# redwarp/kmeans-gpu

Hardware: AMD Instinct MI355X
Metric: pixels/sec per Lloyd iteration (8192x8192, k=256) (higher is better)
Workload: dtype f32; 1 GPU; synthetic uniform RGBA 8192x8192 (seed 0x5EED0003), k=256, one Lloyd iteration = update + assign (labels written every iteration) + accumulate; width=8192, height=8192, k=256, collective_backend=none (one rank), collective_ranks=1, label_pass=before the next iteration, update=by the last launch of the assign pass (kmg_lloyd_assign_update)

## Files before the change

### kmeans-gpu_amd/csrc/kmg_cube.hip

```cpp

#include "kmg_internal.h"
#include "kmg_table_dev.h"

#include <hip/hip_fp16.h>
#include <stdlib.h>

namespace kmg {

typedef float f32x2 __attribute__((ext_vector_type(2)));


namespace {

constexpr uint32_t kMaxListed = 32;
constexpr uint32_t kMaxLong = 256;
constexpr uint32_t kLongFlag = 0x200u;

__device__ __forceinline__ uint32_t sel3(uint32_t i, uint32_t x0, uint32_t x1, uint32_t x2)
{
    return i == 0u ? x0 : (i == 1u ? x1 : x2);
}

__device__ __forceinline__ int round_dir(int g, int m)
{
    const int a = g < 0 ? -g : g;
    const int r = (4 * a >= 3 * m ? 1 : 0) + (4 * a >= m ? 1 : 0);
    return g < 0 ? -r : r;
}

typedef unsigned short u16x2 __attribute__((ext_vector_type(2)));

__device__ __forceinline__ uint32_t group8_or(uint32_t v)
{
    v |= dpp_u32<kDppXor1>(v);
    v |= dpp_u32<kDppXor2>(v);
    v |= dpp_u32<kDppHalfMirror>(v);
    return v;
}

__device__ __forceinline__ uint32_t group8_min_u32(uint32_t v)
{
    v = min(v, dpp_u32<kDppXor1>(v));
    v = min(v, dpp_u32<kDppXor2>(v));
    v = min(v, dpp_u32<kDppHalfMirror>(v));
    return v;
}

__device__ __forceinline__ uint32_t group8_max_u32(uint32_t v)
{
    v = max(v, dpp_u32<kDppXor1>(v));
    v = max(v, dpp_u32<kDppXor2>(v));
    v = max(v, dpp_u32<kDppHalfMirror>(v));
    return v;
}



__device__ __forceinline__ uint32_t cell_pair_entry(const uint32_t idx[8], uint32_t occ, uint32_t lane)
{
    uint32_t rem = occ;
    uint32_t lab0 = 0, lab1 = 0, lab2 = 0, cnt0 = 0, cnt1 = 0, cnt2 = 0, msk0 = 0, msk1 = 0, msk2 = 0, n_occ = 0;
#pragma unroll
    for (int t = 0; t < 3; ++t) {
        const unsigned long long any = __ballot(rem != 0u);
        if (any) {
            uint32_t mine = 0;
#pragma unroll
            for (int q = 7; q >= 0; --q) mine = ((rem >> q) & 1u) ? idx[q] : mine;
            const uint32_t v = lane_value(mine, (uint32_t)__builtin_ctzll(any));
            uint32_t mm = 0;
#pragma unroll
            for (int q = 0; q < 8; ++q) mm |= (idx[q] == v ? 1u : 0u) << q;
            mm &= rem;
            rem &= ~mm;
            const uint32_t packed = wave_add_u32((uint32_t)__builtin_popcount(mm) | (t == 0 ? (uint32_t)__builtin_popcount(occ) << 10 : 0u));
            const uint32_t c = packed & 1023u;
            if (t == 0) { lab0 = v; msk0 = mm; cnt0 = c; n_occ = packed >> 10; }
            if (t == 1) { lab1 = v; msk1 = mm; cnt1 = c; }
            if (t == 2) { lab2 = v; msk2 = mm; cnt2 = c; }
        }
    }
    uint32_t a = 0;
    if (cnt1 > cnt0) a = 1;
    if (cnt2 > sel3(a, cnt0, cnt1, cnt2)) a = 2;
    uint32_t b = a == 0u ? 1u : 0u;
    if (a != 1u && b != 1u && cnt1 > sel3(b, cnt0, cnt1, cnt2)) b = 1;
    if (a != 2u && cnt2 > sel3(b, cnt0, cnt1, cnt2)) b = 2;
    const uint32_t labA = sel3(a, lab0, lab1, lab2), labB = sel3(b, lab0, lab1, lab2);
    const uint32_t mA = sel3(a, msk0, msk1, msk2), mB = sel3(b, msk0, msk1, msk2);
    const uint32_t rest = occ & ~mA;
    const uint32_t nA = sel3(a, cnt0, cnt1, cnt2), nR = n_occ - nA;
    if (nR == 0u) return pair_entry(labA, labA, 0u, 0u, 0u);

    const uint32_t half = ((lane >> 5) & 1u) | (((lane >> 4) & 1u) << 10) | (((lane >> 3) & 1u) << 20);
    const uint32_t hR = wave_add_u32((uint32_t)__builtin_popcount(rest) * half);
    const uint32_t hA = wave_add_u32((uint32_t)__builtin_popcount(mA) * half);
    const int gx = (int)((hR & 1023u) * nA) - (int)((hA & 1023u) * nR);
    const int gy = (int)(((hR >> 10) & 1023u) * nA) - (int)(((hA >> 10) & 1023u) * nR);
    const int gz = (int)((hR >> 20) * nA) - (int)((hA >> 20) * nR);
    const int ax = gx < 0 ? -gx : gx, ay = gy < 0 ? -gy : gy, az = gz < 0 ? -gz : gz;
    const int m = ax > ay ? (ax > az ? ax : az) : (ay > az ? ay : az);
    int nx = 2, ny = 0, nz = 0;
    if (m > 0) { nx = round_dir(gx, m); ny = round_dir(gy, m); nz = round_dir(gz, m); }

    const int xl = (int)(((lane >> 5) & 1u) * 4u + ((lane >> 1) & 3u));
    const int yl = (int)(((lane >> 4) & 1u) * 4u + (lane & 1u) * 2u);
    const int zl = (int)(((lane >> 3) & 1u) * 4u);
    const int bias = 7 * ((nx < 0 ? -nx : 0) + (ny < 0 ? -ny : 0) + (nz < 0 ? -nz : 0));
    const int p0 = nx * xl + ny * yl + nz * zl + bias;
    int p[8];
#pragma unroll
    for (int q = 0; q < 8; ++q) p[q] = p0 + ny * (q >> 2) + nz * (q & 3);
    const uint32_t notB = occ & ~mB;
    uint32_t tl = 63u, hi = 64u;
#pragma unroll
    for (int q = 0; q < 8; ++q) {
        if ((rest >> q) & 1u) tl = min(tl, (uint32_t)p[q]);
        if ((notB >> q) & 1u) hi = min(hi, (uint32_t)(63 - p[q]));
    }
    u16x2 packed = __builtin_bit_cast(u16x2, tl | (hi << 16));
    packed = __builtin_elementwise_min(packed, __builtin_bit_cast(u16x2, dpp_u32<kDppXor1>(__builtin_bit_cast(uint32_t, packed))));
    packed = __builtin_elementwise_min(packed, __builtin_bit_cast(u16x2, dpp_u32<kDppXor2>(__builtin_bit_cast(uint32_t, packed))));
    packed = __builtin_elementwise_min(packed, __builtin_bit_cast(u16x2, dpp_u32<kDppHalfMirror>(__builtin_bit_cast(uint32_t, packed))));
    packed = __builtin_elementwise_min(packed, __builtin_bit_cast(u16x2, dpp_u32<kDppMirror>(__builtin_bit_cast(uint32_t, packed))));
    packed = __builtin_elementwise_min(packed, __builtin_bit_cast(u16x2, (uint32_t)__builtin_amdgcn_update_dpp(-1, (int)__builtin_bit_cast(uint32_t, packed), 0x142, 0xA, 0xF, false)));
    packed = __builtin_elementwise_min(packed, __builtin_bit_cast(u16x2, (uint32_t)__builtin_amdgcn_update_dpp(-1, (int)__builtin_bit_cast(uint32_t, packed), 0x143, 0xC, 0xF, false)));
    const uint32_t pk = lane_value(__builtin_bit_cast(uint32_t, packed), 63);
    const int tlo = (int)(pk & 0xFFFFu);
    const int thi = 63 - (int)(pk >> 16);
    const int w = thi + 1 > tlo ? thi + 1 - tlo : 0;
    const uint32_t code = pair_dir_code(nx, ny, nz);
    if (w <= 6) return pair_entry(labA, labB, code, (uint32_t)tlo, (uint32_t)w);
    uint32_t low = 0, high = 0;
#pragma unroll
    for (int q = 0; q < 8; ++q) {
        if ((occ >> q) & 1u) { low += p[q] < tlo ? 1u : 0u; high += p[q] > thi ? 1u : 0u; }
    }
    const uint32_t lh = wave_add_u32(low | (high << 10));
    if ((lh & 1023u) >= (lh >> 10)) return pair_entry(labA, labB, code, (uint32_t)tlo, 7u);
    const int range = 7 * ((nx < 0 ? -nx : nx) + (ny < 0 ? -ny : ny) + (nz < 0 ? -nz : nz));
    return pair_entry(labB, labA, pair_dir_code(-nx, -ny, -nz), (uint32_t)(range - thi), 7u);
}

__device__ __forceinline__ uint32_t merge_state(uint32_t a, uint32_t b)
{
    return (a == kSubEmpty) ? b : ((b == kSubEmpty || b == a) ? a : (uint32_t)kSubMixed);
}

template <typename LabelT>
__device__ __forceinline__ void store_labels64(LabelT *dst64, uint32_t label, uint32_t lane)
{
    if (sizeof(LabelT) == 1) {
        const uint32_t t = label | (dpp_u32<kDppXor1>(label) << 8);
        const uint32_t u = t | (dpp_u32<kDppXor2>(t) << 16);
        if ((lane & 3u) == 0u) reinterpret_cast<uint32_t *>(dst64)[lane >> 2] = u;
    } else {
        const uint32_t t = label | (dpp_u32<kDppXor1>(label) << 16);
        if ((lane & 1u) == 0u) reinterpret_cast<uint32_t *>(dst64)[lane >> 1] = t;
    }
}


struct alignas(16) CellWork {
    uint16_t list[kMaxListed];
    unsigned long long br[4];
    uint32_t npop;
    uint32_t scan_set;
    uint32_t pad[6];
};
static_assert(sizeof(CellWork) == 128, "CellWork layout");

constexpr uint32_t kPairPending = 0xFFFFFFFEu;

constexpr uint32_t kLongSegs = 16, kLongSegCap = kCells / kLongSegs, kLongCount = 0, kLongCells = 64;
constexpr size_t kListsWords = kLongCells + kCells;
constexpr uint32_t kItemCands = 12;

__device__ __forceinline__ void flush_bins(const unsigned long long *bins, uint32_t k, uint32_t repl, uint32_t bin_stride,
                                           int64_t *sums, uint32_t n_rows)
{
    __syncthreads();
    unsigned long long *row = reinterpret_cast<unsigned long long *>(sums) + (uint64_t)(blockIdx.x % n_rows) * 4ull * k;
    for (uint32_t i = threadIdx.x; i < 4u * k; i += blockDim.x) {
        unsigned long long v = 0ull;
        for (uint32_t r = 0; r < repl; ++r) v += bins[(uint64_t)r * bin_stride + i];
        if (v) atomicAdd(row + i, v);
    }
}

__device__ __forceinline__ uint2 long_list_stage(const float4 *s_cent, const unsigned long long *s_masks, uint16_t *s_long,
                                              unsigned long long *s_sub, float4 sb0, float4 sb1, float4 sb2, uint32_t npop,
                                              uint32_t words, uint64_t *sub_masks_cell)
{
    const uint32_t lane = threadIdx.x & 63u;
    const uint32_t sub_of_lane = lane >> 3, cand_of_lane = lane & 7u;
    uint32_t base = 0;
    for (uint32_t w = 0; w < words; ++w) {
        const unsigned long long m = uniform_u64(s_masks[w]);
        if ((m >> lane) & 1ull) s_long[base + bits_below_lane(m)] = (uint16_t)(w * 64u + lane);
        base += (uint32_t)__builtin_popcountll(m);
    }
    if (lane < 32u) s_sub[lane] = 0ull;
    __builtin_amdgcn_wave_barrier();
    CellBounds sb;
    sb.L0 = sb0.x; sb.L1 = sb0.y; sb.a0 = sb0.z; sb.a1 = sb0.w;
    sb.b0 = sb1.x; sb.b1 = sb1.y; sb.C0 = sb1.z; sb.C1 = sb1.w;
    sb.wC0 = sb2.x; sb.wC1 = sb2.y; sb.wH0 = sb2.z; sb.wH1 = sb2.w;
    const uint32_t rounds = (npop + 7u) >> 3;
    float Usub = 3.0e38f;
    for (uint32_t r = 0; r < rounds; ++r) {
        const uint32_t pos = r * 8u + cand_of_lane;
        if (pos < npop) {
            const float4 c = s_cent[s_long[pos]];
            Usub = fminf(Usub, key_range(sb, c.x, c.y, c.z, c.w).hi);
        }
    }
    const float Us = mask_threshold(group8_min(Usub));
    for (uint32_t r = 0; r < rounds; ++r) {
        const uint32_t pos = r * 8u + cand_of_lane;
        if (pos < npop) {
            const uint32_t j = s_long[pos];
            const float4 c = s_cent[j];
            if (key_range(sb, c.x, c.y, c.z, c.w).lo <= Us) atomicOr(&s_sub[sub_of_lane * 4u + (j >> 6)], 1ull << (j & 63u));
        }
    }
    __builtin_amdgcn_wave_barrier();
    const unsigned long long mine = lane < 32u ? s_sub[lane] : 0ull;
    if (lane < 32u) sub_masks_cell[lane] = mine;
    uint32_t cnt = (uint32_t)__builtin_popcountll(mine);
    uint32_t one = mine ? (lane & 3u) * 64u + (uint32_t)__builtin_ctzll(mine) : 0u;
    cnt += dpp_u32<kDppXor1>(cnt); one += dpp_u32<kDppXor1>(one);
    cnt += dpp_u32<kDppXor2>(cnt); one += dpp_u32<kDppXor2>(one);
    uint2 r;
    r.x = (uint32_t)__builtin_amdgcn_ds_bpermute((int)((lane * 4u) << 2), (int)cnt);
    r.y = (uint32_t)__builtin_amdgcn_ds_bpermute((int)((lane * 4u) << 2), (int)one);
    return r;
}


constexpr uint32_t kAffineFloats = 24;
struct HalfModel {
    uint32_t q[kAffineFloats];
    __device__ __forceinline__ float operator[](int i) const
    {
        if (i >= 42) return bits_to_float(q[21 + (i - 42)]);
        const uint32_t h = (i & 1) ? q[i >> 1] >> 16 : q[i >> 1] & 0xFFFFu;
        return __half2float(__ushort_as_half((unsigned short)h));
    }
    __device__ __forceinline__ void load(const float *table, uint64_t sub_cell)
    {
        const uint4 *mp = reinterpret_cast<const uint4 *>(table + sub_cell * kAffineFloats);
#pragma unroll
        for (int t = 0; t < 6; ++t) {
            const uint4 v = mp[t];
            q[4 * t] = v.x; q[4 * t + 1] = v.y; q[4 * t + 2] = v.z; q[4 * t + 3] = v.w;
// ... 484 lines not shown
                }
                const float thr0 = tie_threshold(best0), thr1 = tie_threshold(best1);
                const bool near0 = second0 <= thr0, near1 = second1 <= thr1;
                if (__ballot(near0 || near1)) {
                    float lb0 = 100000.0f, lb1 = 100000.0f;
                    uint32_t li0 = 0u, li1 = 0u;
                    for (uint32_t w = 0; w < (k + 63u) / 64u; ++w) {
                        for (unsigned long long m = cand_word(w); m; m &= m - 1ull) {
                            const uint32_t j = w * 64u + (uint32_t)__builtin_ctzll(m);
                            const float4 c = s_cent[j];
                            if (near0 && cie94_key(pt0, c.x, c.y, c.z, c.w) <= thr0) {
                                const float d = cie94_c(v0.x, v0.y, v0.z, v0.w, c.x, c.y, c.z, c.w);
                                if (d < lb0) { lb0 = d; li0 = j; }
                            }
                            if (near1 && cie94_key(pt1, c.x, c.y, c.z, c.w) <= thr1) {
                                const float d = cie94_c(v1.x, v1.y, v1.z, v1.w, c.x, c.y, c.z, c.w);
                                if (d < lb1) { lb1 = d; li1 = j; }
                            }
                        }
                    }
                    ix0 = near0 ? li0 : ix0;
                    ix1 = near1 ? li1 : ix1;
                }
            }
            auto finish = [&](uint32_t s, uint32_t ix, uint32_t cnt, float vL, float va, float vb) {
                s_lbl[s * 64u + lane] = (LabelT)ix;
                label_set |= 1u << s;
                const bool counts = cnt != 0u;
                const unsigned long long occm = __ballot(counts);
                uint32_t st = kSubEmpty;
                if (occm) {
                    const uint32_t X0 = lane_value(ix, (uint32_t)__builtin_ctzll(occm));
                    const unsigned long long other = __ballot(counts && ix != X0);
                    uint32_t R = X0;
                    if (other) {
                        const uint32_t X1 = lane_value(ix, (uint32_t)__builtin_ctzll(other));
                        if (__builtin_popcountll(__ballot(counts && ix == X1)) > __builtin_popcountll(occm & ~other)) R = X1;
                    }
                    st = other ? (uint32_t)kSubMixed : X0;
                    if (SUMS) {
                        if ((lane >> 2) == s) atomicAdd(bins + 4ull * R + (lane & 3u), (unsigned long long)sagg);
                        if (other && counts && ix != R) {
                            const long long m = (long long)cnt;
                            const long long c0 = m * (long long)lab_fix(vL), c1 = m * (long long)lab_fix(va), c2 = m * (long long)lab_fix(vb);
                            unsigned long long *to = my_bins + 4ull * ix, *from = my_bins + 4ull * R;
                            atomicAdd(to + 0, (unsigned long long)c0); atomicAdd(from + 0, (unsigned long long)(-c0));
                            atomicAdd(to + 1, (unsigned long long)c1); atomicAdd(from + 1, (unsigned long long)(-c1));
                            atomicAdd(to + 2, (unsigned long long)c2); atomicAdd(from + 2, (unsigned long long)(-c2));
                            atomicAdd(to + 3, (unsigned long long)m);  atomicAdd(from + 3, (unsigned long long)(-m));
                        }
                    }
                }
                if (sizeof(LabelT) != 1 && lane == 0u) sub[s] = (uint16_t)st;
            };
            finish(s0, ix0, cnt0, v0.x, v0.y, v0.z);
            if (s1 < 8u) finish(s1, ix1, cnt1, v1.x, v1.y, v1.z);
        };
        for (;;) {
            KMG_REQUEST_COLOURS(B);
            scan_pair(A_s0, A_s1, A_v0, A_v1, A_c0, A_c1);
            if (B_s0 >= 8u) break;
            KMG_REQUEST_COLOURS(A);
            scan_pair(B_s0, B_s1, B_v0, B_v1, B_c0, B_c1);
            if (A_s0 >= 8u) break;
        }
#undef KMG_REQUEST_COLOURS
        __builtin_amdgcn_wave_barrier();
        if ((label_set >> (lane >> 3)) & 1u) {
            if (sizeof(LabelT) == 1)
                *reinterpret_cast<uint2 *>(cell_labels + lane * 8u) = *reinterpret_cast<const uint2 *>(s_lbl + lane * 8u);
            else
                *reinterpret_cast<uint4 *>(cell_labels + lane * 8u) = *reinterpret_cast<const uint4 *>(s_lbl + lane * 8u);
        }
        __builtin_amdgcn_wave_barrier();
    }
    if (SUMS) flush_bins(bins, k, repl, bin_stride, sums, n_rows);
}

template <typename LabelT>
__global__ __launch_bounds__(kBlock) void k_cube_pairs(const uint32_t *__restrict__ work, int with_work,
                                                       const uint8_t *__restrict__ occ_bits,
                                                       const LabelT *__restrict__ colour_labels,
                                                       uint16_t *__restrict__ sub_table, uint32_t flags,
                                                       int64_t *__restrict__ sums, uint32_t k, CubeTail tail)
{
    if (tail.acc_out && blockIdx.x == gridDim.x - 1u) {
        __shared__ uint32_t s_count;
        for (uint32_t i = threadIdx.x; i < 4u * k; i += kBlock) tail.acc_out[i] = sums[i];
        if (tail.do_update) update_centroids(sums, k, tail.convergence, tail.cent, tail.n_converged, &s_count, kBlock);
        __syncthreads();
        for (uint32_t i = threadIdx.x; i < 4u * k; i += kBlock) sums[i] = 0;
    }
    if (flags & kCubeNoEntries) return;
    const uint32_t lane = threadIdx.x & 63;
    const uint32_t wave = __builtin_amdgcn_readfirstlane(blockIdx.x * (kBlock / 64) + (threadIdx.x >> 6));
    const uint32_t n_waves = gridDim.x * (kBlock / 64);
    const uint32_t n_work = with_work ? __builtin_amdgcn_readfirstlane(work[0]) : kCells;
    const uint32_t *cells = with_work ? work + 1 : nullptr;
    for (uint32_t wi = wave; wi < n_work; wi += n_waves) {
        const uint32_t cell = cells ? __builtin_amdgcn_readfirstlane(cells[wi]) : wi;
        if (sizeof(LabelT) == 1) {
            uint32_t *pair_entry_ptr = reinterpret_cast<uint32_t *>(sub_table + kSubCells + kCells) + cell;
            if (__builtin_amdgcn_readfirstlane(*pair_entry_ptr) != kPairPending) continue;
            const uint2 lv = *reinterpret_cast<const uint2 *>(colour_labels + (uint64_t)cell * kCellColours + lane * 8u);
            const uint32_t occ = occ_bits ? (uint32_t)occ_bits[(uint64_t)cell * 64u + lane] : 0xFFu;
            uint32_t idx[8];
#pragma unroll
            for (uint32_t q = 0; q < 4u; ++q) { idx[q] = (lv.x >> (8u * q)) & 0xFFu; idx[4u + q] = (lv.y >> (8u * q)) & 0xFFu; }
            const uint32_t e = cell_pair_entry(idx, occ, lane);
            if (lane == 0u) *pair_entry_ptr = e;
        } else {
            uint32_t st = lane < 8u ? (uint32_t)sub_table[cell * 8u + lane] : (uint32_t)kSubEmpty;
#pragma unroll
            for (int off = 1; off < 8; off <<= 1) st = merge_state(st, (uint32_t)__shfl_xor(st, off, 64));
            if (lane == 0u) sub_table[kSubCells + cell] = (uint16_t)st;
        }
    }
}

constexpr uint32_t kSmallMaxK = kCubeSmallMaxK;
constexpr uint32_t kSmallRepl = 16;
constexpr int kSmallBlock = 512;
constexpr uint32_t kSmallWaves = kSmallBlock / 64;
constexpr uint32_t kSmallCells = kSmallWaves * 8u;
constexpr uint32_t kSmallEmit = 0x100u;
constexpr uint32_t kSmallTests = 2048;

__device__ __forceinline__ void affine_features(const float4 v, double F[7])
{
    const PixelTerms p = pixel_terms_c(v.x, v.y, v.z, v.w);
    F[0] = (double)p.L; F[1] = (double)p.wC; F[2] = (double)p.wC * (double)p.C;
    F[3] = (double)p.wH * (double)p.a; F[4] = (double)p.wH * (double)p.b; F[5] = (double)p.wH * (double)p.C; F[6] = (double)p.wH;
}

__global__ __launch_bounds__(kBlock) void k_sub_affine(const float4 *__restrict__ lab_table,
                                                       const CellBounds *__restrict__ sub_bounds, float *__restrict__ affine)
{
    const uint32_t sc = blockIdx.x * kBlock + threadIdx.x;
    if (sc >= kSubCells) return;
    const float4 *col = lab_table + (uint64_t)sc * 64u;
    double S0[7], Sx[7], Sy[7], Sz[7];
#pragma unroll
    for (int m = 0; m < 7; ++m) S0[m] = Sx[m] = Sy[m] = Sz[m] = 0.0;
    for (uint32_t q = 0; q < 64u; ++q) {
        double F[7];
        affine_features(col[q], F);
        const double dx = (double)((q >> 4) & 3u) - 1.5, dy = (double)((q >> 2) & 3u) - 1.5, dz = (double)(q & 3u) - 1.5;
#pragma unroll
        for (int m = 0; m < 7; ++m) { S0[m] += F[m]; Sx[m] += F[m] * dx; Sy[m] += F[m] * dy; Sz[m] += F[m] * dz; }
    }
    float al[7], bx[7], by[7], bz[7];
    double rmin[7], rmax[7];
#pragma unroll
    for (int m = 0; m < 7; ++m) {
        al[m] = __half2float(__float2half_rn((float)(S0[m] / 64.0))); bx[m] = __half2float(__float2half_rn((float)(Sx[m] / 80.0)));
        by[m] = __half2float(__float2half_rn((float)(Sy[m] / 80.0))); bz[m] = __half2float(__float2half_rn((float)(Sz[m] / 80.0)));
        rmin[m] = 1.0e300; rmax[m] = -1.0e300;
    }
    for (uint32_t q = 0; q < 64u; ++q) {
        double F[7];
        affine_features(col[q], F);
        const double dx = (double)((q >> 4) & 3u) - 1.5, dy = (double)((q >> 2) & 3u) - 1.5, dz = (double)(q & 3u) - 1.5;
#pragma unroll
        for (int m = 0; m < 7; ++m) {
            const double r = F[m] - ((double)al[m] + ((double)bx[m] * dx + ((double)by[m] * dy + (double)bz[m] * dz)));
            rmin[m] = fmin(rmin[m], r); rmax[m] = fmax(rmax[m], r);
        }
    }
    uint32_t *out = reinterpret_cast<uint32_t *>(affine) + (uint64_t)sc * kAffineFloats;
    unsigned short h[42];
#pragma unroll
    for (int m = 0; m < 7; ++m) {
        const double pad = 1.0e-12 * (fabs((double)al[m]) + 1.5 * (fabs((double)bx[m]) + fabs((double)by[m]) + fabs((double)bz[m])) + 1.0);
        const double lo = rmin[m] - pad, hi = rmax[m] + pad;
        float flo = (float)lo, fhi = (float)hi;
        if ((double)flo > lo) flo = nextafterf(flo, -3.0e38f);
        if ((double)fhi < hi) fhi = nextafterf(fhi, 3.0e38f);
        h[6 * m + 0] = __half_as_ushort(__float2half_rn(al[m])); h[6 * m + 1] = __half_as_ushort(__float2half_rn(bx[m]));
        h[6 * m + 2] = __half_as_ushort(__float2half_rn(by[m])); h[6 * m + 3] = __half_as_ushort(__float2half_rn(bz[m]));
        h[6 * m + 4] = __half_as_ushort(__float2half_rd(flo)); h[6 * m + 5] = __half_as_ushort(__float2half_ru(fhi));
    }
#pragma unroll
    for (int w = 0; w < 21; ++w) out[w] = (uint32_t)h[2 * w] | ((uint32_t)h[2 * w + 1] << 16);
    out[21] = float_to_bits(sub_bounds[sc].C1);
    out[22] = float_to_bits(sub_bounds[sc].wH1);
    out[23] = 0u;
}

size_t sub_affine_bytes() { return sizeof(float) * (size_t)kAffineFloats * kSubCells; }

hipError_t launch_sub_affine(const float4 *lab_table, const CellBounds *sub_bounds, float *affine, hipStream_t st)
{
    hipLaunchKernelGGL(k_sub_affine, dim3(kSubCells / kBlock), dim3(kBlock), 0, st, lab_table, sub_bounds, affine);
    return hipGetLastError();
}

template <int KP, bool SUMS>
__global__ __launch_bounds__(kSmallBlock) __attribute__((amdgpu_waves_per_eu(4, 4))) void k_cube_small(const uint32_t *__restrict__ hist, const int64_t *__restrict__ agg,
                                                            const int64_t *__restrict__ sub_agg,
                                                            const uint8_t *__restrict__ occ_bits,
                                                            const uint32_t *__restrict__ work,
                                                            const CellBounds *__restrict__ bounds,
                                                            const CellBounds *__restrict__ sub_bounds,
                                                            const float *__restrict__ sub_affine,
                                                            const Centroid *__restrict__ cent, uint32_t k,
                                                            const float4 *__restrict__ lab_table,
                                                            uint64_t *__restrict__ masks_out,
                                                            CellWork *__restrict__ cell_work,
                                                            uint8_t *__restrict__ colour_labels,
                                                            uint16_t *__restrict__ sub_table,
                                                            int64_t *__restrict__ sums, uint32_t n_rows, uint32_t flags,
                                                            unsigned long long *__restrict__ stats)
{
    extern __shared__ float4 smem4[];
    float4 *s_cent = smem4;
    unsigned long long *bins = reinterpret_cast<unsigned long long *>(smem4 + KP);
    const uint32_t bin_stride = 4u * k + 4u;
    const uint32_t n_bins = SUMS ? kSmallRepl * bin_stride : 0u;
    uint8_t *s_lbl = reinterpret_cast<uint8_t *>(bins + n_bins);
    uint32_t *s_mask = reinterpret_cast<uint32_t *>(s_lbl + kSmallCells * kCellColours);
    float *s_U = reinterpret_cast<float *>(s_mask + kSmallBlock);
    uint32_t *s_cell = reinterpret_cast<uint32_t *>(s_U + kSmallBlock);
    uint32_t *s_count = s_cell + kSmallCells;
    uint16_t *s_ent = reinterpret_cast<uint16_t *>(s_count + 4);
    uint16_t *s_pend = s_ent + kSmallBlock;
    uint16_t *s_test = s_pend + kSmallCells;
    uint8_t *s_istar = reinterpret_cast<uint8_t *>(s_test + kSmallTests);
    const uint32_t n_work_v = SUMS ? work[opaque_vgpr_zero()] : kCells;
    for (uint32_t i = threadIdx.x; i < (uint32_t)KP; i += kSmallBlock) {
        float4 v = make_float4(1.0e18f, 0.0f, 0.0f, 0.0f);
        if (i < k) { const Centroid c = cent[i]; v = make_float4(c.L, c.a, c.b, c.C); }
        s_cent[i] = v;
    }
    for (uint32_t i = threadIdx.x; i < n_bins; i += kSmallBlock) bins[i] = 0ull;
    if (threadIdx.x < 4u) s_count[threadIdx.x] = 0u;
    __syncthreads();
    if (threadIdx.x < k) {
        const float4 c = s_cent[threadIdx.x];
        if (!(fabsf(c.x) <= 1024.0f && fabsf(c.y) <= 1024.0f && fabsf(c.z) <= 1024.0f)) s_count[2] = 1u;
    }
    __syncthreads();
    const bool dominance = sub_affine != nullptr && s_count[2] == 0u;

    const uint32_t lane = threadIdx.x & 63u, wv = threadIdx.x >> 6;
    unsigned long long *my_bins = bins + (uint64_t)(lane & (kSmallRepl - 1u)) * bin_stride;
    uint32_t *pair_entries = reinterpret_cast<uint32_t *>(sub_table + kSubCells + kCells);
    const uint32_t ci = lane >> 3, sub = lane & 7u, slot = wv * 8u + ci;
    unsigned long long st_single = 0, st_multi = 0, st_decided = 0, st_scanned = 0, st_cands = 0;

    const uint32_t n_work = __builtin_amdgcn_readfirstlane(n_work_v);
    const uint32_t tasks = (n_work + 7u) >> 3;
    for (uint32_t base = blockIdx.x * kSmallWaves; base < tasks; base += gridDim.x * kSmallWaves) {
        const uint32_t task = base + wv;
        const uint32_t pos = task + ci * tasks;
        const bool valid = task < tasks && pos < n_work;
        const uint32_t cell = valid ? ((SUMS && n_work != kCells) ? work[1u + pos] : pos) : 0u;
        const uint32_t sc = cell * 8u + sub;
        const float4 *cbp = reinterpret_cast<const float4 *>(bounds + cell);
        const float4 cb0 = cbp[0], cb1 = cbp[1], cb2 = cbp[2];
        const float4 *sbp = reinterpret_cast<const float4 *>(sub_bounds + sc);
        const float4 sb0 = sbp[0], sb1 = sbp[1], sb2 = sbp[2];
        longlong2 s01 = {0, 0}, s23 = {0, 1};
        long long cell_sum = 0;
        if (SUMS) {
            const longlong2 *sp = reinterpret_cast<const longlong2 *>(sub_agg + (uint64_t)sc * 4u);
            s01 = sp[0]; s23 = sp[1];
            cell_sum = agg[4ull * cell + (sub & 3u)];
        }
        const bool occupied = valid && s23.y != 0;
        uint32_t mask = 0u;
        {
            CellBounds cb;
            cb.L0 = cb0.x; cb.L1 = cb0.y; cb.a0 = cb0.z; cb.a1 = cb0.w;
            cb.b0 = cb1.x; cb.b1 = cb1.y; cb.C0 = cb1.z; cb.C1 = cb1.w;
            cb.wC0 = cb2.x; cb.wC1 = cb2.y; cb.wH0 = cb2.z; cb.wH1 = cb2.w;
            constexpr int PER = KP / 8;
            float lo[PER], Uc = 3.0e38f;
#pragma unroll
            for (int q = 0; q < PER; ++q) {
                const float4 c = s_cent[sub * PER + q];
                const KeyRange kr = key_range(cb, c.x, c.y, c.z, c.w);
                lo[q] = kr.lo;
                Uc = fminf(Uc, kr.hi);
            }
            const float Ucs = mask_threshold(group8_min(Uc));
            uint32_t bits = 0u;
#pragma unroll
            for (int q = 0; q < PER; ++q) bits |= (lo[q] <= Ucs ? 1u : 0u) << (sub * PER + q);
            const uint32_t cmask = group8_or(bits);
            CellBounds sb;
            sb.L0 = sb0.x; sb.L1 = sb0.y; sb.a0 = sb0.z; sb.a1 = sb0.w;
            sb.b0 = sb1.x; sb.b1 = sb1.y; sb.C0 = sb1.z; sb.C1 = sb1.w;
            sb.wC0 = sb2.x; sb.wC1 = sb2.y; sb.wH0 = sb2.z; sb.wH1 = sb2.w;
            float U = 3.0e38f;
            uint32_t istar = 0u;
            for (uint32_t m = cmask; m; m &= m - 1u) {
                const uint32_t j = (uint32_t)__builtin_ctz(m);
                const float4 c = s_cent[j];
                const float hi = key_range(sb, c.x, c.y, c.z, c.w).hi;
                istar = hi < U ? j : istar;
                U = fminf(U, hi);
            }
            const float Us = mask_threshold(U);
            for (uint32_t m = cmask; m; m &= m - 1u) {
                const uint32_t j = (uint32_t)__builtin_ctz(m);
                const float4 c = s_cent[j];
                mask |= (key_range(sb, c.x, c.y, c.z, c.w).lo <= Us ? 1u : 0u) << j;
            }
            s_mask[threadIdx.x] = mask;
            const uint32_t others = mask & ~(1u << istar);
            if (dominance && occupied && others) {
                s_U[threadIdx.x] = U;
                s_istar[threadIdx.x] = (uint8_t)istar;
                const uint32_t nt = (uint32_t)__builtin_popcount(others);
                uint32_t at = atomicAdd(&s_count[3], nt);
                for (uint32_t m = others; m && at < kSmallTests; m &= m - 1u, ++at)
                    s_test[at] = (uint16_t)((threadIdx.x << 5) | (uint32_t)__builtin_ctz(m));
            }
        }
        if (sub == 0u) s_cell[slot] = cell;
        __syncthreads();
        if (dominance) {
            const uint32_t n_tests = min(s_count[3], kSmallTests);
            for (uint32_t t = threadIdx.x; t < n_tests; t += kSmallBlock) {
                const uint32_t e = (uint32_t)s_test[t] >> 5, j = (uint32_t)s_test[t] & 31u;
                const uint32_t tsc = s_cell[e >> 3] * 8u + (e & 7u);
                HalfModel mdl;
                mdl.load(sub_affine, tsc);
                if (dominated(mdl, s_cent[j], s_cent[s_istar[e]], s_U[e])) atomicAnd(&s_mask[e], ~(1u << j));
            }
            __syncthreads();
            mask = s_mask[threadIdx.x];
        }

        const uint32_t np = (uint32_t)__builtin_popcount(mask);
        const bool decided = occupied && np == 1u, scan = occupied && np > 1u;
        const uint32_t X = (uint32_t)__builtin_ctz(mask | 0x80000000u);
        const uint32_t um = group8_or(mask);
        const uint32_t any_scan = group8_or(scan ? 1u : 0u);
        const uint32_t xmin = group8_min_u32(decided ? X : 255u), xmax = group8_max_u32(decided ? X : 0u);
        const bool uniform = valid && !any_scan && xmin == xmax;
        if (valid && sub == 0u) masks_out[cell] = (uint64_t)um;
        if (SUMS) {
            if (uniform) {
                if (sub < 4u) atomicAdd(my_bins + 4ull * xmin + sub, (unsigned long long)cell_sum);
            } else if (decided) {
                unsigned long long *to = my_bins + 4ull * X;
                atomicAdd(to + 0, (unsigned long long)s01.x); atomicAdd(to + 1, (unsigned long long)s01.y);
                atomicAdd(to + 2, (unsigned long long)s23.x); atomicAdd(to + 3, (unsigned long long)s23.y);
            }
        }
        {
            const uint32_t x4 = (decided ? X : 0u) * 0x01010101u;
            const uint4 xv = make_uint4(x4, x4, x4, x4);
            if (uniform) {
                if (sub == 0u) pair_entries[cell] = pair_entry(xmin, xmin, 0u, 0u, 0u);
                if (flags & 1u) {
                    const uint32_t m4 = xmin * 0x01010101u;
                    uint4 *dst = reinterpret_cast<uint4 *>(colour_labels + (uint64_t)cell * kCellColours + sub * 64u);
                    dst[0] = dst[1] = dst[2] = dst[3] = make_uint4(m4, m4, m4, m4);
                }
            } else if (valid && !(flags & kSmallEmit)) {
                uint4 *dst = reinterpret_cast<uint4 *>(s_lbl + slot * kCellColours + sub * 64u);
                dst[0] = xv; dst[1] = xv; dst[2] = xv; dst[3] = xv;
            } else if (valid && decided) {
                uint4 *dst = reinterpret_cast<uint4 *>(colour_labels + (uint64_t)cell * kCellColours + sub * 64u);
                dst[0] = xv; dst[1] = xv; dst[2] = xv; dst[3] = xv;
            }
        }
        if (flags & kSmallEmit) {
            if (valid) {
                CellWork *cw = cell_work + cell;
                const uint32_t scan8 = group8_or(scan ? 1u << sub : 0u);
                uint32_t lo_w[4], hi_w[4];
#pragma unroll
                for (uint32_t r = 0; r < 4u; ++r) {
                    const uint32_t byte = (mask >> (8u * r)) & 0xFFu;
                    lo_w[r] = group8_or(sub < 4u ? byte << (8u * sub) : 0u);
                    hi_w[r] = group8_or(sub >= 4u ? byte << (8u * (sub - 4u)) : 0u);
                }
                if (sub < 4u) {
                    const uint32_t l = sub == 0u ? lo_w[0] : (sub == 1u ? lo_w[1] : (sub == 2u ? lo_w[2] : lo_w[3]));
                    const uint32_t h = sub == 0u ? hi_w[0] : (sub == 1u ? hi_w[1] : (sub == 2u ? hi_w[2] : hi_w[3]));
                    cw->br[sub] = ((unsigned long long)h << 32) | l;
                }
                const uint32_t p0 = 4u * sub;
                *reinterpret_cast<uint2 *>(cw->list + p0) = make_uint2(p0 | (p0 + 1u) << 16, (p0 + 2u) | (p0 + 3u) << 16);
                if (sub == 0u) {
                    cw->npop = uniform ? 1u : k;
                    cw->scan_set = uniform ? 0u : (scan8 | 0x100u);
                    if (!uniform) pair_entries[cell] = kPairPending;
                }
            }
            if (stats) {
                const unsigned long long scan_b = __ballot(scan);
                st_single += (uint32_t)__builtin_popcountll(__ballot(valid && sub == 0u && __builtin_popcount(um) == 1));
                st_multi += (uint32_t)__builtin_popcountll(__ballot(valid && sub == 0u && __builtin_popcount(um) != 1));
                st_decided += (uint32_t)__builtin_popcountll(__ballot(decided && __builtin_popcount(um) != 1));
                st_scanned += (uint32_t)__builtin_popcountll(scan_b);
                st_cands += wave_add_u32(scan ? np : 0u);
            }
            __syncthreads();
            if (threadIdx.x == 3u) s_count[3] = 0u;
            __syncthreads();
            continue;
        }
        {
            const unsigned long long scan_b = __ballot(scan);
            const unsigned long long pend_b = __ballot(valid && !uniform && sub == 0u);
            uint32_t e_base = 0u, p_base = 0u;
            if (lane == 0u) {
                if (scan_b) e_base = atomicAdd(&s_count[0], (uint32_t)__builtin_popcountll(scan_b));
                if (pend_b) p_base = atomicAdd(&s_count[1], (uint32_t)__builtin_popcountll(pend_b));
            }
            e_base = __builtin_amdgcn_readfirstlane(e_base);
            p_base = __builtin_amdgcn_readfirstlane(p_base);
            if (scan) s_ent[e_base + bits_below_lane(scan_b)] = (uint16_t)threadIdx.x;
            if (valid && !uniform && sub == 0u) s_pend[p_base + bits_below_lane(pend_b)] = (uint16_t)slot;
            if (stats) {
                const unsigned long long single_b = __ballot(valid && sub == 0u && __builtin_popcount(um) == 1);
                const unsigned long long multi_b = __ballot(valid && sub == 0u && __builtin_popcount(um) != 1);
                const unsigned long long dec_b = __ballot(decided && __builtin_popcount(um) != 1);
                st_single += (uint32_t)__builtin_popcountll(single_b);
                st_multi += (uint32_t)__builtin_popcountll(multi_b);
                st_decided += (uint32_t)__builtin_popcountll(dec_b);
                st_scanned += (uint32_t)__builtin_popcountll(scan_b);
                st_cands += wave_add_u32(scan ? np : 0u);
            }
        }
        __syncthreads();
        const uint32_t n_ent = s_count[0];
        const uint32_t n_pend = s_count[1];

        uint32_t occ_early[2] = {0xFFu, 0xFFu};
        if (occ_bits && !(flags & kCubeNoEntries)) {
#pragma unroll
            for (uint32_t q = 0; q < 2u; ++q) {
                const uint32_t pi = wv + q * kSmallWaves;
                if (pi < n_pend) occ_early[q] = (uint32_t)occ_bits[(uint64_t)s_cell[s_pend[pi]] * 64u + lane];
// ... 45 lines not shown
                    asm("v_bfi_b32 %0, 31, %1, %2" : "=v"(u0) : "s"(pos), "v"(float_to_bits(key.x)));
                    asm("v_bfi_b32 %0, 31, %1, %2" : "=v"(u1) : "s"(pos), "v"(float_to_bits(key.y)));
                    r0 = umed3(u0, b0, r0); b0 = min(b0, u0);
                    r1 = umed3(u1, b1, r1); b1 = min(b1, u1);
                }
                uint32_t p0 = b0 & 31u, p1 = b1 & 31u;
                const float thr0 = tie_threshold(bits_to_float(b0 & ~31u)), thr1 = tie_threshold(bits_to_float(b1 & ~31u));
                const bool near0 = bits_to_float(r0 & ~31u) <= thr0, near1 = bits_to_float(r1 & ~31u) <= thr1;
                if (__ballot(near0 || near1)) {
                    float lb0 = 100000.0f, lb1 = 100000.0f;
                    uint32_t li0 = 0u, li1 = 0u;
                    for (uint32_t m = sm; m; m &= m - 1u) {
                        const uint32_t pos = (uint32_t)__builtin_ctz(m);
                        const float4 c = s_cent[pos];
                        if (near0 && cie94_key(pt0, c.x, c.y, c.z, c.w) <= thr0) {
                            const float d = cie94_c(v0.x, v0.y, v0.z, v0.w, c.x, c.y, c.z, c.w);
                            if (d < lb0) { lb0 = d; li0 = pos; }
                        }
                        if (near1 && cie94_key(pt1, c.x, c.y, c.z, c.w) <= thr1) {
                            const float d = cie94_c(v1.x, v1.y, v1.z, v1.w, c.x, c.y, c.z, c.w);
                            if (d < lb1) { lb1 = d; li1 = pos; }
                        }
                    }
                    p0 = near0 ? li0 : p0;
                    p1 = near1 ? li1 : p1;
                }
                auto finish = [&](uint32_t e, uint32_t ix, uint32_t cnt, long long g, float vL, float va, float vb) {
                    s_lbl[(e >> 3) * kCellColours + (e & 7u) * 64u + lane] = (uint8_t)ix;
                    if (!SUMS) return;
                    const bool counts = cnt != 0u;
                    const unsigned long long occm = __ballot(counts);
                    if (!occm) return;
                    const uint32_t X0 = lane_value(ix, (uint32_t)__builtin_ctzll(occm));
                    const unsigned long long other = __ballot(counts && ix != X0);
                    uint32_t R = X0;
                    if (other) {
                        const uint32_t X1 = lane_value(ix, (uint32_t)__builtin_ctzll(other));
                        if (__builtin_popcountll(__ballot(counts && ix == X1)) > __builtin_popcountll(occm & ~other)) R = X1;
                    }
                    if (lane < 4u) atomicAdd(my_bins + 4ull * R + lane, (unsigned long long)g);
                    if (other && counts && ix != R) {
                        const long long m = (long long)cnt;
                        const long long c0 = m * (long long)lab_fix(vL), c1 = m * (long long)lab_fix(va), c2 = m * (long long)lab_fix(vb);
                        unsigned long long *to = my_bins + 4ull * ix, *from = my_bins + 4ull * R;
                        atomicAdd(to + 0, (unsigned long long)c0); atomicAdd(from + 0, (unsigned long long)(-c0));
                        atomicAdd(to + 1, (unsigned long long)c1); atomicAdd(from + 1, (unsigned long long)(-c1));
                        atomicAdd(to + 2, (unsigned long long)c2); atomicAdd(from + 2, (unsigned long long)(-c2));
                        atomicAdd(to + 3, (unsigned long long)m);  atomicAdd(from + 3, (unsigned long long)(-m));
                    }
                };
                finish(e0, p0, cnt0, g0, v0.x, v0.y, v0.z);
                if (has1) finish(e1, p1, cnt1, g1, v1.x, v1.y, v1.z);
            };
            KMG_REQUEST_PAIR(A);
            KMG_REQUEST_PAIR(B);
            KMG_REQUEST_PAIR(C);
            for (;;) {
                scan_pair(A_e0, A_e1, A_h1, A_v0, A_v1, A_c0, A_c1, A_g0, A_g1);
                if (!B_ok) break;
                KMG_REQUEST_PAIR(A);
                scan_pair(B_e0, B_e1, B_h1, B_v0, B_v1, B_c0, B_c1, B_g0, B_g1);
                if (!C_ok) break;
                KMG_REQUEST_PAIR(B);
                scan_pair(C_e0, C_e1, C_h1, C_v0, C_v1, C_c0, C_c1, C_g0, C_g1);
                if (!A_ok) break;
                KMG_REQUEST_PAIR(C);
            }
#undef KMG_REQUEST_PAIR
        }
        __syncthreads();

        for (uint32_t pi = wv; pi < n_pend; pi += kSmallWaves) {
            const uint32_t ps = __builtin_amdgcn_readfirstlane((uint32_t)s_pend[pi]);
            const uint32_t pcell = __builtin_amdgcn_readfirstlane(s_cell[ps]);
            const uint2 lv = *reinterpret_cast<const uint2 *>(s_lbl + ps * kCellColours + lane * 8u);
            uint32_t e = kPairPending;
            if (!(flags & kCubeNoEntries)) {
                const uint32_t round = (pi - wv) / kSmallWaves;
                const uint32_t occ = round == 0u ? occ_early[0] : (round == 1u ? occ_early[1] :
                                     (occ_bits ? (uint32_t)occ_bits[(uint64_t)pcell * 64u + lane] : 0xFFu));
                uint32_t idx[8];
#pragma unroll
                for (uint32_t q = 0; q < 4u; ++q) { idx[q] = (lv.x >> (8u * q)) & 0xFFu; idx[4u + q] = (lv.y >> (8u * q)) & 0xFFu; }
                e = cell_pair_entry(idx, occ, lane);
            }
            if (lane == 0u) pair_entries[pcell] = e;
            *reinterpret_cast<uint2 *>(colour_labels + (uint64_t)pcell * kCellColours + lane * 8u) = lv;
        }
        __syncthreads();
        if (threadIdx.x < 2u) s_count[threadIdx.x] = 0u;
        if (threadIdx.x == 3u) s_count[3] = 0u;
        __syncthreads();
    }
    if (stats && lane == 0u) {
        atomicAdd(stats + 0, st_single); atomicAdd(stats + 1, st_multi); atomicAdd(stats + 2, st_decided);
        atomicAdd(stats + 3, st_scanned); atomicAdd(stats + 4, st_cands);
    }
    if (SUMS) {
        __syncthreads();
        unsigned long long *row = reinterpret_cast<unsigned long long *>(sums) + (uint64_t)(blockIdx.x % n_rows) * 4ull * k;
        for (uint32_t i = threadIdx.x; i < 4u * k; i += kSmallBlock) {
            unsigned long long v = 0ull;
            for (uint32_t r = 0; r < kSmallRepl; ++r) v += bins[(uint64_t)r * bin_stride + i];
            if (v) atomicAdd(row + i, v);
        }
    }
}

constexpr int kOneBlock = 1024;
constexpr uint32_t kOneWaves = kOneBlock / 64, kOneCells = kOneWaves * 8u;
constexpr uint32_t kOneItems = kOneCells * 4u;
constexpr uint32_t kOneTests = 384;
constexpr uint32_t kOneRepl = 4;

constexpr uint32_t kOneTaskSlots = (kCells / kOneCells) * kOneWaves;
constexpr uint32_t kOneBalWords = 80;
size_t cube_balance_bytes() { return sizeof(uint16_t) * 4u * kOneTaskSlots; }

static size_t cube_one_lds_bytes(uint32_t k, bool with_sums)
{
    const size_t bins = with_sums ? sizeof(unsigned long long) * kOneRepl * (4ull * k + 4ull) : 0u;
    return sizeof(float4) * 256u + bins + (size_t)kOneCells * kCellColours + sizeof(uint4) * kOneItems + sizeof(uint16_t) * kOneWaves * kOneTests +
           sizeof(unsigned long long) * kOneCells * 4u + sizeof(uint32_t) * kOneBlock * 2u + (size_t)kOneCells * 64u +
           sizeof(uint32_t) * kOneCells * 3u + sizeof(uint32_t) * (8u + kOneWaves + kOneBalWords) + sizeof(uint16_t) * kOneCells * kMaxListed;
}

#ifdef KMG_TOOLS
__device__ unsigned long long g_one_stamps[(kCells / kOneCells) * 12u];
#define KMG_STAMP(i) do { if (threadIdx.x == 0u) g_one_stamps[blockIdx.x * 12u + (i)] = wall_clock64(); } while (0)
#define KMG_STAMP_VALUE(i, v) do { if (threadIdx.x == 0u) g_one_stamps[blockIdx.x * 12u + (i)] = (v); } while (0)
#else
#define KMG_STAMP(i) do { } while (0)
#define KMG_STAMP_VALUE(i, v) do { } while (0)
#endif

template <bool SUMS>
__global__ __launch_bounds__(kOneBlock) __attribute__((amdgpu_waves_per_eu(4, 4))) void k_cube_one(
    const uint32_t *__restrict__ hist, const int64_t *__restrict__ agg, const int64_t *__restrict__ sub_agg,
    const uint8_t *__restrict__ occ_bits, const uint32_t *__restrict__ work, const CellBounds *__restrict__ bounds,
    const CellBounds *__restrict__ sub_bounds, const float *__restrict__ sub_affine, const Centroid *__restrict__ cent, uint32_t k,
    const float4 *__restrict__ lab_table, uint64_t *__restrict__ masks_out, uint8_t *__restrict__ colour_labels,
    uint16_t *__restrict__ sub_table, int64_t *__restrict__ sums, uint32_t n_rows, uint32_t flags,
    unsigned long long *__restrict__ stats, uint16_t *__restrict__ bal_state, uint32_t bal_pass)
{
    extern __shared__ float4 smem4[];
    float4 *s_cent = smem4;
    unsigned long long *bins = reinterpret_cast<unsigned long long *>(smem4 + 256);
    const uint32_t bin_stride = 4u * k + 4u;
    const uint32_t n_bins = SUMS ? kOneRepl * bin_stride : 0u;
    uint8_t *s_lbl = reinterpret_cast<uint8_t *>(bins + n_bins);
    uint4 *s_item = reinterpret_cast<uint4 *>(s_lbl + kOneCells * kCellColours);
    uint16_t *s_test = reinterpret_cast<uint16_t *>(s_item + kOneItems);
    unsigned long long *s_cmask = reinterpret_cast<unsigned long long *>(s_test + kOneWaves * kOneTests);
    uint32_t *s_mask = reinterpret_cast<uint32_t *>(s_cmask + kOneCells * 4u);
    uint32_t *s_ref = s_mask + kOneBlock;
    uint8_t *s_occ = reinterpret_cast<uint8_t *>(s_ref + kOneBlock);
    uint32_t *s_cell = reinterpret_cast<uint32_t *>(s_occ + kOneCells * 64u);
    uint32_t *s_npop = s_cell + kOneCells;
    uint32_t *s_left = s_npop + kOneCells;
    uint32_t *s_count = s_left + kOneCells;
    uint32_t *s_bal = s_count + 8 + kOneWaves;
    uint16_t *s_list = reinterpret_cast<uint16_t *>(s_bal + kOneBalWords);

    const uint32_t vz = opaque_vgpr_zero();
    const uint32_t n_work_v = SUMS ? work[vz] : kCells;
    if (threadIdx.x < 256u) {
        float4 v = make_float4(1.0e18f, 0.0f, 0.0f, 0.0f);
        if (threadIdx.x < k) { const Centroid c = cent[threadIdx.x]; v = make_float4(c.L, c.a, c.b, c.C); }
        s_cent[threadIdx.x] = v;
    }
    if (threadIdx.x < 8u + kOneWaves) s_count[threadIdx.x] = 0u;
    if (SUMS) for (uint32_t i = threadIdx.x; i < n_bins; i += kOneBlock) bins[i] = 0ull;
    if (bal_state && (threadIdx.x >> 6) == kOneWaves - 1u) {
        const uint32_t bl = threadIdx.x & 63u;
        const uint32_t nw = __builtin_amdgcn_readfirstlane(n_work_v);
        const uint32_t bcpw = min(8u, max(1u, (nw + gridDim.x * kOneWaves - 1u) / (gridDim.x * kOneWaves)));
        const uint32_t btasks = (nw + bcpw - 1u) / bcpw, bused = (btasks + gridDim.x - 1u) / gridDim.x;
        uint16_t *cur = bal_state + (bal_pass & 1u) * 2u * kOneTaskSlots;
        const uint16_t *prev = bal_state + ((bal_pass + 1u) & 1u) * 2u * kOneTaskSlots;
        uint32_t id = 0xFFFFu;
        if (bal_pass == 0u) {
            if (bl < bused && blockIdx.x * bused + bl < btasks) id = blockIdx.x * bused + bl;
        } else {
            const uint32_t partner = blockIdx.x ^ (1u << ((bal_pass - 1u) & 7u));
            const uint32_t lo_wg = min(blockIdx.x, partner), hi_wg = max(blockIdx.x, partner);
            const uint32_t src = ((bl & 16u) ? hi_wg : lo_wg) * kOneWaves + (bl & 15u);
            uint32_t e_id = 0xFFFFu, e_w = 0u;
            if (bl < 32u) { e_id = prev[src]; e_w = prev[kOneTaskSlots + src]; }
            if (e_id >= btasks) { e_id = 0xFFFFu; e_w = 0u; }
            if (bl < 32u) s_bal[bl] = (e_w << 16) | e_id;
            __builtin_amdgcn_wave_barrier();
            uint32_t rank = 0;
            for (uint32_t j = 0; j < 32u; ++j) {
                const uint32_t ow = s_bal[j] >> 16;
                rank += (ow > e_w || (ow == e_w && j < bl)) ? 1u : 0u;
            }
            if (bl < 32u) s_bal[32u + rank] = (e_w << 16) | e_id;
            __builtin_amdgcn_wave_barrier();
            const uint32_t sorted = bl < 32u ? s_bal[32u + bl] : 0u;
            const bool i_am_hi = blockIdx.x == hi_wg;
            uint32_t t0 = 0, t1 = 0, c0 = 0, c1 = 0;
#pragma unroll
            for (uint32_t r = 0; r < 32u; ++r) {
                const uint32_t e = lane_value(sorted, r);
                const bool to_hi = c0 >= kOneWaves || (c1 < kOneWaves && t1 < t0);
                if (to_hi) { if (i_am_hi && bl == c1) id = e & 0xFFFFu; ++c1; t1 += e >> 16; }
                else       { if (!i_am_hi && bl == c0) id = e & 0xFFFFu; ++c0; t0 += e >> 16; }
            }
        }
        if (bl < kOneWaves) { cur[blockIdx.x * kOneWaves + bl] = (uint16_t)id; s_bal[64u + bl] = id; }
    }
    __syncthreads();
    if (threadIdx.x < k) {
        const float4 c = s_cent[threadIdx.x];
        if (!(fabsf(c.x) <= 1024.0f && fabsf(c.y) <= 1024.0f && fabsf(c.z) <= 1024.0f)) s_count[2] = 1u;
    }
    __syncthreads();
    const bool dominance = sub_affine != nullptr && s_count[2] == 0u;

    const uint32_t lane = threadIdx.x & 63u, wv = threadIdx.x >> 6;
    const uint32_t ci = lane >> 3, sub = lane & 7u, slot = wv * 8u + ci;
    unsigned long long *my_bins = bins + (uint64_t)(lane & (kOneRepl - 1u)) * bin_stride;
    uint32_t *pair_entries = reinterpret_cast<uint32_t *>(sub_table + kSubCells + kCells);
    const uint32_t words = (k + 63u) / 64u;
    unsigned long long st_single = 0, st_multi = 0, st_unlisted = 0, st_decided = 0, st_scanned = 0, st_cands = 0, st_removed = 0, st_one = 0;
    float4 c4[4];
// ... 79 lines not shown

        const uint32_t np_first = s_npop[slot];
        const uint32_t npop = valid ? (np_first & 0xFFFFu) : 1u, first = np_first >> 16;
        const bool listed = valid && npop > 1u && npop <= kMaxListed;
        const bool unlisted = valid && npop > kMaxListed;
        const bool occupied = valid && (SUMS ? g23.y != 0 : true);
        uint32_t sm = 0u, istar = 0u, ubits = 0u;
        if (listed) {
            CellBounds sb;
            sb.L0 = sb0.x; sb.L1 = sb0.y; sb.a0 = sb0.z; sb.a1 = sb0.w;
            sb.b0 = sb1.x; sb.b1 = sb1.y; sb.C0 = sb1.z; sb.C1 = sb1.w;
            sb.wC0 = sb2.x; sb.wC1 = sb2.y; sb.wH0 = sb2.z; sb.wH1 = sb2.w;
            uint32_t Ubest = 0x7F7FFFE0u;
            for (uint32_t p = 0; p < npop; ++p) {
                const float4 c = s_cent[s_list[slot * kMaxListed + p]];
                Ubest = min(Ubest, ((float_to_bits(key_range(sb, c.x, c.y, c.z, c.w).hi) + 31u) & ~31u) | p);
            }
            const float Us = mask_threshold(bits_to_float(Ubest & ~31u));
            for (uint32_t p = 0; p < npop; ++p) {
                const float4 c = s_cent[s_list[slot * kMaxListed + p]];
                sm |= (key_range(sb, c.x, c.y, c.z, c.w).lo <= Us ? 1u : 0u) << p;
            }
            istar = Ubest & 31u;
            ubits = Ubest & ~31u;
        }
        const uint32_t np0 = (uint32_t)__builtin_popcount(sm);
        const bool was_decided = listed && occupied && np0 == 1u;
        const bool mine = listed && occupied && np0 > 1u;
        s_mask[threadIdx.x] = sm;
        *reinterpret_cast<uint2 *>(s_occ + slot * 64u + sub * 8u) = occ8;
        const uint32_t others = (mine && dominance) ? sm & ~(1u << istar) : 0u;
        if (others) {
            s_ref[threadIdx.x] = ubits | istar;
            const uint32_t nt = (uint32_t)__builtin_popcount(others);
            uint32_t at = atomicAdd(&s_count[8u + wv], nt);
            for (uint32_t m = others; m && at < kOneTests; m &= m - 1u, ++at)
                s_test[wv * kOneTests + at] = (uint16_t)((lane << 5) | (uint32_t)__builtin_ctz(m));
        }
        KMG_STAMP(2);
        __builtin_amdgcn_fence(__ATOMIC_RELEASE, "workgroup");
        __builtin_amdgcn_wave_barrier();
        __builtin_amdgcn_fence(__ATOMIC_ACQUIRE, "workgroup");
        if (dominance) {
            const uint32_t n_tests = min(__builtin_amdgcn_readfirstlane(s_count[8u + wv]), kOneTests);
            for (uint32_t t = lane; t < n_tests; t += 64u) {
                const uint32_t ent = (uint32_t)s_test[wv * kOneTests + t];
                const uint32_t e = wv * 64u + (ent >> 5), tp = ent & 31u;
                const uint32_t r = s_ref[e];
                const float4 cj = s_cent[s_list[(e >> 3) * kMaxListed + tp]], ci4 = s_cent[s_list[(e >> 3) * kMaxListed + (r & 31u)]];
                HalfModel mdl;
                mdl.load(sub_affine, (uint64_t)s_cell[e >> 3] * 8u + (e & 7u));
                if (dominated(mdl, cj, ci4, bits_to_float(r & ~31u))) atomicAnd(&s_mask[e], ~(1u << tp));
            }
            __builtin_amdgcn_fence(__ATOMIC_RELEASE, "workgroup");
            __builtin_amdgcn_wave_barrier();
            __builtin_amdgcn_fence(__ATOMIC_ACQUIRE, "workgroup");
        }
        KMG_STAMP(3);

        const uint32_t nm = s_mask[threadIdx.x];
        const uint32_t np = (uint32_t)__builtin_popcount(nm);
        const bool one = mine && np == 1u, still = mine && np > 1u;
        const uint32_t X = listed ? (uint32_t)s_list[slot * kMaxListed + (nm ? (uint32_t)__builtin_ctz(nm) : 0u)] : first;
        const bool open = still || (unlisted && occupied);
        const uint32_t scan8 = group8_or(open ? 1u << sub : 0u);
        const bool settled = one || was_decided;
        const uint32_t xmin = group8_min_u32(settled ? X : 255u), xmax = group8_max_u32(settled ? X : 0u);
        const bool single = valid && npop == 1u;
        const bool uniform = single || (listed && scan8 == 0u && xmin == xmax);
        const uint32_t Xu = single ? first : xmin;
        if (SUMS) {
            if (uniform) {
                if (sub < 4u) atomicAdd(my_bins + 4ull * Xu + sub, (unsigned long long)cell_sum);
            } else if (settled) {
                unsigned long long *to = my_bins + 4ull * X;
                atomicAdd(to + 0, (unsigned long long)g01.x); atomicAdd(to + 1, (unsigned long long)g01.y);
                atomicAdd(to + 2, (unsigned long long)g23.x); atomicAdd(to + 3, (unsigned long long)g23.y);
            }
        }
        {
            const uint32_t x4 = (settled ? X : 0u) * 0x01010101u;
            const uint4 xv = make_uint4(x4, x4, x4, x4);
            if (uniform) {
                if (sub == 0u) pair_entries[cell] = pair_entry(Xu, Xu, 0u, 0u, 0u);
                if (flags & 1u) {
                    const uint32_t m4 = Xu * 0x01010101u;
                    uint4 *dst = reinterpret_cast<uint4 *>(colour_labels + (uint64_t)cell * kCellColours + sub * 64u);
                    dst[0] = dst[1] = dst[2] = dst[3] = make_uint4(m4, m4, m4, m4);
                }
            } else if (valid) {
                uint4 *dst = reinterpret_cast<uint4 *>(s_lbl + slot * kCellColours + sub * 64u);
                dst[0] = xv; dst[1] = xv; dst[2] = xv; dst[3] = xv;
            }
        }
        unsigned long long pend0_b = 0ull;
        {
            const uint32_t rank = (uint32_t)__builtin_popcount(scan8 & ((1u << sub) - 1u));
            const bool head = open && (rank & 1u) == 0u;
            const uint32_t after = scan8 & ~((2u << sub) - 1u);
            const uint32_t s1 = after ? (uint32_t)__builtin_ctz(after) : 8u;
            const uint32_t un = listed ? (nm | ((head && s1 < 8u) ? s_mask[threadIdx.x - sub + s1] : 0u)) : 0u;
            const uint32_t n_un = (uint32_t)__builtin_popcount(un);
            const uint32_t type = unlisted ? 2u : (n_un > kItemCands ? 1u : 0u);
            const bool pend = valid && !uniform && sub == 0u;
            if (pend) s_left[slot] = ((uint32_t)__builtin_popcount(scan8) + 1u) >> 1;
            pend0_b = __ballot(pend && scan8 == 0u);
            const unsigned long long item_b = __ballot(head);
            if (bal_state) {
                const uint32_t cost = wave_add_u32(head ? 4u + (type == 2u ? npop : n_un) : 0u);
                if (lane == 0u) bal_state[(bal_pass & 1u) * 2u * kOneTaskSlots + kOneTaskSlots + blockIdx.x * kOneWaves + wv] = (uint16_t)min(cost, 65535u);
            }
            uint32_t i_base = 0u;
            if (lane == 0u && item_b) i_base = atomicAdd(&s_count[0], (uint32_t)__builtin_popcountll(item_b));
            i_base = __builtin_amdgcn_readfirstlane(i_base);
            if (head) {
                uint32_t iw0 = un, iw1 = 0u, iw2 = 0u;
                if (type == 0u) {
                    iw0 = 0u;
                    uint32_t q = 0u;
                    for (uint32_t m = un; m; m &= m - 1u, ++q) {
                        const uint32_t cc = (uint32_t)s_list[slot * kMaxListed + (uint32_t)__builtin_ctz(m)] << (8u * (q & 3u));
                        iw0 |= q < 4u ? cc : 0u; iw1 |= (q >= 4u && q < 8u) ? cc : 0u; iw2 |= q >= 8u ? cc : 0u;
                    }
                }
                s_item[i_base + bits_below_lane(item_b)] = make_uint4(slot | (sub << 7) | (s1 << 10) | (n_un << 14) | (type << 30), iw0, iw1, iw2);
            }
            if (stats) {
                st_single += (uint32_t)__builtin_popcountll(__ballot(single && sub == 0u));
                st_multi += (uint32_t)__builtin_popcountll(__ballot(valid && !single && sub == 0u));
                st_unlisted += (uint32_t)__builtin_popcountll(__ballot(unlisted && sub == 0u));
                st_decided += (uint32_t)__builtin_popcountll(__ballot(was_decided));
                st_scanned += (uint32_t)__builtin_popcountll(__ballot(mine || (unlisted && occupied)));
                st_cands += wave_add_u32(mine ? np0 : ((unlisted && occupied) ? npop : 0u));
                st_removed += wave_add_u32((uint32_t)__builtin_popcount(sm & ~nm));
                st_one += (uint32_t)__builtin_popcountll(__ballot(one));
            }
        }
        KMG_STAMP(4);
        __syncthreads();
        const uint32_t n_items = s_count[0];
        KMG_STAMP_VALUE(8, n_items); KMG_STAMP_VALUE(10, s_count[8]);

        auto cell_entry = [&](const uint32_t ps) {
            const uint32_t pcell = __builtin_amdgcn_readfirstlane(s_cell[ps]);
            const uint2 lv = *reinterpret_cast<const uint2 *>(s_lbl + ps * kCellColours + lane * 8u);
            uint32_t e = kPairPending;
            if (!(flags & kCubeNoEntries)) {
                const uint32_t occ = (uint32_t)s_occ[ps * 64u + lane];
                uint32_t idx[8];
#pragma unroll
                for (uint32_t q = 0; q < 4u; ++q) { idx[q] = (lv.x >> (8u * q)) & 0xFFu; idx[4u + q] = (lv.y >> (8u * q)) & 0xFFu; }
                e = cell_pair_entry(idx, occ, lane);
            }
            if (lane == 0u) pair_entries[pcell] = e;
            *reinterpret_cast<uint2 *>(colour_labels + (uint64_t)pcell * kCellColours + lane * 8u) = lv;
        };

        {
            uint32_t A_h = 0u, A_w0 = 0u, A_w1 = 0u, A_w2 = 0u, B_h = 0u, B_w0 = 0u, B_w1 = 0u, B_w2 = 0u, C_h = 0u, C_w0 = 0u, C_w1 = 0u, C_w2 = 0u;
            float4 A_v0, A_v1, B_v0, B_v1, C_v0, C_v1;
            uint32_t A_c0 = 1u, A_c1 = 1u, B_c0 = 1u, B_c1 = 1u, C_c0 = 1u, C_c1 = 1u;
            long long A_g = 0, B_g = 0, C_g = 0;
            bool A_ok = false, B_ok = false, C_ok = false;
#define KMG_REQUEST_ITEM(X)                                                                                       \
            do {                                                                                                  \
                uint32_t next_ = 0u;                                                                              \
                if (lane == 0u) next_ = atomicAdd(&s_count[4], 1u);                                               \
                next_ = __builtin_amdgcn_readfirstlane(next_);                                                    \
                X##_ok = next_ < n_items;                                                                         \
                const uint4 it_ = s_item[next_ < n_items ? next_ : 0u];                                           \
                X##_h = __builtin_amdgcn_readfirstlane(it_.x); X##_w0 = __builtin_amdgcn_readfirstlane(it_.y);    \
                X##_w1 = __builtin_amdgcn_readfirstlane(it_.z); X##_w2 = __builtin_amdgcn_readfirstlane(it_.w);   \
                const uint32_t cell_ = __builtin_amdgcn_readfirstlane(s_cell[X##_h & 127u]);                       \
                const uint32_t c0_ = cell_ * kCellColours + ((X##_h >> 7) & 7u) * 64u + lane;                     \
                const uint32_t c1_ = cell_ * kCellColours + ((X##_h >> 10) & 7u) * 64u + lane;    \
                X##_v0 = lab_table[c0_]; X##_v1 = lab_table[c1_];                                                 \
                if (SUMS) { X##_c0 = hist[c0_]; X##_c1 = hist[c1_]; X##_g = sub_agg[(uint64_t)cell_ * 32u + (lane & 31u)]; } \
            } while (0)
            auto scan_item = [&](const uint32_t hdr, const uint32_t w0, const uint32_t w1, const uint32_t w2, const float4 v0, const float4 v1,
                                 const uint32_t cnt0, const uint32_t cnt1, const long long sagg) {
                const uint32_t islot = hdr & 127u, s0 = (hdr >> 7) & 7u, s1 = (hdr >> 10) & 15u, n = (hdr >> 14) & 63u, type = hdr >> 30;
                const PixelTerms pt0 = pixel_terms_fast(v0.x, v0.y, v0.z, v0.w), pt1 = pixel_terms_fast(v1.x, v1.y, v1.z, v1.w);
                uint32_t ix0 = 0u, ix1 = 0u;
                if (type == 0u) {
                    const uint32_t my_cand = ((lane < 4u ? w0 : (lane < 8u ? w1 : w2)) >> (8u * (lane & 3u))) & 0xFFu;
                    uint32_t b0 = 0x7F7FFFFFu, r0 = 0x7F7FFFFFu, b1 = 0x7F7FFFFFu, r1 = 0x7F7FFFFFu;
                    const f32x2 qL = {pt0.L, pt1.L}, qa = {pt0.a, pt1.a}, qb = {pt0.b, pt1.b}, qC = {pt0.C, pt1.C};
                    const f32x2 qwC = {pt0.wC, pt1.wC}, qwH = {pt0.wH, pt1.wH};
                    auto cand_at = [&](uint32_t p) { return ((p < 4u ? w0 : (p < 8u ? w1 : w2)) >> (8u * (p & 3u))) & 0xFFu; };
                    for (uint32_t p = 0; p < n; ++p) {
                        const float4 c = s_cent[cand_at(p)];
                        const f32x2 dL = qL - c.x, da = qa - c.y, db = qb - c.z, dC = qC - c.w;
                        const f32x2 dC2 = dC * dC;
                        const f32x2 t = __builtin_elementwise_fma(db, db, da * da);
                        f32x2 h = t - dC2;
                        h.x = fmaxf(h.x, 0.0f); h.y = fmaxf(h.y, 0.0f);
                        const f32x2 key = __builtin_elementwise_fma(h, qwH, __builtin_elementwise_fma(dC2, qwC, dL * dL));
                        uint32_t u0, u1;
                        asm("v_bfi_b32 %0, 31, %1, %2" : "=v"(u0) : "s"(p), "v"(float_to_bits(key.x)));
                        asm("v_bfi_b32 %0, 31, %1, %2" : "=v"(u1) : "s"(p), "v"(float_to_bits(key.y)));
                        r0 = umed3(u0, b0, r0); b0 = min(b0, u0);
                        r1 = umed3(u1, b1, r1); b1 = min(b1, u1);
                    }
                    uint32_t p0 = b0 & 31u, p1 = b1 & 31u;
                    const float thr0 = tie_threshold(bits_to_float(b0 & ~31u)), thr1 = tie_threshold(bits_to_float(b1 & ~31u));
                    const bool near0 = bits_to_float(r0 & ~31u) <= thr0, near1 = bits_to_float(r1 & ~31u) <= thr1;
                    if (__ballot(near0 || near1)) {
                        float lb0 = 100000.0f, lb1 = 100000.0f;
                        uint32_t li0 = 0u, li1 = 0u;
                        for (uint32_t p = 0; p < n; ++p) {
                            const float4 c = s_cent[cand_at(p)];
                            if (near0 && cie94_key(pt0, c.x, c.y, c.z, c.w) <= thr0) {
                                const float d = cie94_c(v0.x, v0.y, v0.z, v0.w, c.x, c.y, c.z, c.w);
                                if (d < lb0) { lb0 = d; li0 = p; }
                            }
                            if (near1 && cie94_key(pt1, c.x, c.y, c.z, c.w) <= thr1) {
                                const float d = cie94_c(v1.x, v1.y, v1.z, v1.w, c.x, c.y, c.z, c.w);
                                if (d < lb1) { lb1 = d; li1 = p; }
                            }
                        }
                        p0 = near0 ? li0 : p0;
                        p1 = near1 ? li1 : p1;
                    }
                    ix0 = (uint32_t)__builtin_amdgcn_ds_bpermute((int)(p0 << 2), (int)my_cand);
                    ix1 = (uint32_t)__builtin_amdgcn_ds_bpermute((int)(p1 << 2), (int)my_cand);
                } else {
                    float best0 = 1.0e10f, second0 = 1.0e10f, best1 = 1.0e10f, second1 = 1.0e10f;
                    const uint32_t rounds = type == 1u ? 1u : words;
                    auto cand_word = [&](uint32_t w) -> unsigned long long { return type == 1u ? (unsigned long long)w0 : uniform_u64(s_cmask[islot * 4u + w]); };
                    auto cand_of = [&](uint32_t w, uint32_t bit) -> uint32_t {
                        return type == 1u ? __builtin_amdgcn_readfirstlane((uint32_t)s_list[islot * kMaxListed + bit]) : w * 64u + bit;
                    };
                    for (uint32_t w = 0; w < rounds; ++w) {
                        for (unsigned long long m = cand_word(w); m; m &= m - 1ull) {
                            const uint32_t j = cand_of(w, (uint32_t)__builtin_ctzll(m));
// ... 44 lines not shown
                    if ((lane >> 2) == s) atomicAdd(bins + 4ull * R + (lane & 3u), (unsigned long long)sagg);
                    if (other && counts && ix != R) {
                        const long long m = (long long)cnt;
                        const long long c0 = m * (long long)lab_fix(vL), c1 = m * (long long)lab_fix(va), c2 = m * (long long)lab_fix(vb);
                        unsigned long long *to = my_bins + 4ull * ix, *from = my_bins + 4ull * R;
                        atomicAdd(to + 0, (unsigned long long)c0); atomicAdd(from + 0, (unsigned long long)(-c0));
                        atomicAdd(to + 1, (unsigned long long)c1); atomicAdd(from + 1, (unsigned long long)(-c1));
                        atomicAdd(to + 2, (unsigned long long)c2); atomicAdd(from + 2, (unsigned long long)(-c2));
                        atomicAdd(to + 3, (unsigned long long)m);  atomicAdd(from + 3, (unsigned long long)(-m));
                    }
                };
                finish(s0, ix0, cnt0, v0.x, v0.y, v0.z);
                if (s1 < 8u) finish(s1, ix1, cnt1, v1.x, v1.y, v1.z);
                __builtin_amdgcn_fence(__ATOMIC_RELEASE, "workgroup");
                uint32_t left = 0u;
                if (lane == 0u) left = atomicSub(&s_left[islot], 1u);
                left = __builtin_amdgcn_readfirstlane(left);
                if (left == 1u) {
                    __builtin_amdgcn_fence(__ATOMIC_ACQUIRE, "workgroup");
                    cell_entry(islot);
                }
            };
            KMG_REQUEST_ITEM(A);
            KMG_REQUEST_ITEM(B);
            KMG_REQUEST_ITEM(C);
            for (;;) {
                if (!A_ok) break;
                scan_item(A_h, A_w0, A_w1, A_w2, A_v0, A_v1, A_c0, A_c1, A_g);
                if (!B_ok) break;
                KMG_REQUEST_ITEM(A);
                scan_item(B_h, B_w0, B_w1, B_w2, B_v0, B_v1, B_c0, B_c1, B_g);
                if (!C_ok) break;
                KMG_REQUEST_ITEM(B);
                scan_item(C_h, C_w0, C_w1, C_w2, C_v0, C_v1, C_c0, C_c1, C_g);
                KMG_REQUEST_ITEM(C);
            }
#undef KMG_REQUEST_ITEM
        }
        KMG_STAMP(5);
        for (unsigned long long m = pend0_b; m; m &= m - 1ull) cell_entry(wv * 8u + ((uint32_t)__builtin_ctzll(m) >> 3));
        KMG_STAMP(7);
    }
    if (stats && lane == 0u) {
        atomicAdd(stats + 0, st_single); atomicAdd(stats + 1, st_multi); atomicAdd(stats + 2, st_decided); atomicAdd(stats + 3, st_scanned);
        atomicAdd(stats + 4, st_cands); atomicAdd(stats + 5, st_unlisted); atomicAdd(stats + 6, st_removed); atomicAdd(stats + 7, st_one);
    }
    if (SUMS) flush_bins(bins, k, kOneRepl, bin_stride, sums, n_rows);
}

#ifdef KMG_TOOLS
extern "C" KMG_API int kmg_tools_cube_one_stamps(unsigned long long *out, uint32_t n)
try {
    return (int)hipMemcpyFromSymbol(out, HIP_SYMBOL(g_one_stamps), sizeof(unsigned long long) * std::min<size_t>(n, (kCells / kOneCells) * 12u));
}
KMG_ABI_CATCH
#endif

static uint32_t grid_or(const char *e, uint32_t dflt)
{
    if (e) { const int v = atoi(e); if (v >= 1 && v <= 65536) return (uint32_t)v; }
    return dflt;
}
#define env_grid(name, dflt) grid_or(KMG_TOOLS_ENV(name), (dflt))

uint32_t cube_replicas(uint32_t k)
{
    uint32_t r = 4;
    if (const char *e = KMG_TOOLS_ENV("KMG_CUBE_REPL")) { const int v = atoi(e); if (v == 1 || v == 2 || v == 4 || v == 8) r = (uint32_t)v; }
    while (r > 1u && (uint64_t)r * (k * 32ull + 32ull) > 33024ull) r >>= 1;
    return r;
}

size_t cube_work_bytes() { return sizeof(CellWork) * (size_t)kCells + sizeof(uint32_t) * kListsWords; }

bool cube_single_launch(uint32_t k, uint32_t flags)
{
    return k <= kSmallMaxK || (k <= 256u && !(flags & kCubeHot));
}

hipError_t launch_cube(const uint32_t *hist, const int64_t *agg, const int64_t *sub_agg, const uint8_t *occ_bits,
                       const uint32_t *work, const CellBounds *bounds, const CellBounds *sub_bounds, const Centroid *cent,
                       uint32_t k, const float4 *lab_table, uint64_t *masks, void *cell_work, void *colour_labels,
                       uint16_t *sub_table, int64_t *sums, uint32_t n_rows, uint32_t flags, unsigned long long *stats,
                       hipStream_t st, const CubeTail *tail, const float *sub_affine, const CubeBalance *balance)
{
    const CubeTail tl = (tail && hist && n_rows <= 1u) ? *tail : CubeTail();
    const uint32_t kpad = (k + 63u) & ~63u;
    const bool with_sums = hist != nullptr;
    const uint32_t repl = with_sums ? cube_replicas(k) : 1u;
    const size_t lds_stage = sizeof(float4) * kpad + (with_sums ? sizeof(unsigned long long) * 4ull * k : 0) +
                             sizeof(uint32_t) * (kBlock / 64) * kMaxListed + sizeof(unsigned long long) * (kBlock / 64) * (kpad / 64u) +
                             (k <= 256 ? (kBlock / 64) * (32u * sizeof(unsigned long long) + kMaxLong * sizeof(uint16_t)) : 0u);
    const size_t lds_scan = sizeof(float4) * kpad + (with_sums ? sizeof(unsigned long long) * (4ull * k + 4ull) * repl : 0) +
                            sizeof(float4) * (kScanBlock / 64) * kMaxListed + (k <= 256 ? 1u : 2u) * (kScanBlock / 64) * kCellColours;
    {
        const size_t lds_max = device_info().lds_max;
        if (lds_stage > lds_max || lds_scan > lds_max) return hipErrorInvalidValue;
    }
    const size_t lds_max_dev = device_info().lds_max;
    static const bool small_on = tools_env_int(KMG_TOOLS_ENV("KMG_CUBE_SMALL"), 1) != 0;
    if (k <= kSmallMaxK && small_on) {
        static const uint32_t g_small = env_grid("KMG_SMALL_GRID", kCells / kSmallCells);
        const uint32_t kp = k <= 8u ? 8u : (k <= 16u ? 16u : 32u);
        const size_t lds = sizeof(float4) * kp + (with_sums ? sizeof(unsigned long long) * (4ull * k + 4ull) * kSmallRepl : 0) +
                           (size_t)kSmallCells * kCellColours + sizeof(uint32_t) * kSmallBlock * 2u + sizeof(uint32_t) * kSmallCells +
                           sizeof(uint32_t) * 4u + sizeof(uint16_t) * (kSmallBlock + kSmallCells + kSmallTests) + kSmallBlock;
        if (!n_rows) n_rows = 1u;
        static const bool split = tools_env_int(KMG_TOOLS_ENV("KMG_CUBE_SMALL"), 1) == 2;
        const uint32_t sflags = (flags & ~0x100u) | (split ? kSmallEmit : 0u);
#define KMG_SMALL(KP, S)                                                                                                    \
        hipLaunchKernelGGL((k_cube_small<KP, S>), dim3(g_small), dim3(kSmallBlock), lds, st, hist, agg, sub_agg, occ_bits,   \
                           work, bounds, sub_bounds, sub_affine, cent, k, lab_table, masks, (CellWork *)cell_work,            \
                           (uint8_t *)colour_labels, sub_table, sums, n_rows, sflags, stats)
        if (with_sums) { if (kp == 8u) KMG_SMALL(8, true); else if (kp == 16u) KMG_SMALL(16, true); else KMG_SMALL(32, true); }
        else           { if (kp == 8u) KMG_SMALL(8, false); else if (kp == 16u) KMG_SMALL(16, false); else KMG_SMALL(32, false); }
#undef KMG_SMALL
        if (split) {
            static const uint32_t g_scan2 = env_grid("KMG_SCAN_GRID", kCubeGrid), g_pairs2 = env_grid("KMG_PAIRS_GRID", kCubeGrid);
            const uint32_t kpad2 = (k + 63u) & ~63u, repl2 = with_sums ? cube_replicas(k) : 1u;
            const size_t lds_scan2 = sizeof(float4) * kpad2 + (with_sums ? sizeof(unsigned long long) * (4ull * k + 4ull) * repl2 : 0) +
                                     sizeof(float4) * (kScanBlock / 64) * kMaxListed + (kScanBlock / 64) * kCellColours;
            if (with_sums)
                hipLaunchKernelGGL((k_cube_scan<uint8_t, true>), dim3(g_scan2), dim3(kScanBlock), lds_scan2, st, hist, sub_agg, work, cent, k,
                                   lab_table, masks, (const CellWork *)cell_work, (uint8_t *)colour_labels, sub_table, sums, n_rows, repl2, flags);
            else
                hipLaunchKernelGGL((k_cube_scan<uint8_t, false>), dim3(g_scan2), dim3(kScanBlock), lds_scan2, st, hist, sub_agg, work, cent, k,
                                   lab_table, masks, (const CellWork *)cell_work, (uint8_t *)colour_labels, sub_table, sums, n_rows, repl2, flags);
            hipLaunchKernelGGL((k_cube_pairs<uint8_t>), dim3((flags & kCubeNoEntries) ? 1u : g_pairs2), dim3(kBlock), 0, st, work,
                               with_sums ? 1 : 0, occ_bits, (const uint8_t *)colour_labels, sub_table, flags, sums, k, tl);
            return hipGetLastError();
        }
        if (tl.acc_out)
            hipLaunchKernelGGL((k_cube_pairs<uint8_t>), dim3(1), dim3(kBlock), 0, st, work, 1, occ_bits,
                               (const uint8_t *)colour_labels, sub_table, flags | kCubeNoEntries, sums, k, tl);
        return hipGetLastError();
    }
    if (cube_single_launch(k, flags)) {
        const size_t lds = cube_one_lds_bytes(k, with_sums);
        if (lds > lds_max_dev) return hipErrorInvalidValue;
        if (!n_rows) n_rows = 1u;
        static const bool balance_on = tools_env_int(KMG_TOOLS_ENV("KMG_BALANCE"), 1) != 0;
        if (!balance_on) balance = nullptr;
        if (with_sums)
            hipLaunchKernelGGL((k_cube_one<true>), dim3(kCells / kOneCells), dim3(kOneBlock), lds, st, hist, agg, sub_agg, occ_bits, work, bounds,
                               sub_bounds, sub_affine, cent, k, lab_table, masks, (uint8_t *)colour_labels, sub_table, sums, n_rows, flags, stats,
                               balance ? balance->state : nullptr, balance ? balance->pass : 0u);
        else
            hipLaunchKernelGGL((k_cube_one<false>), dim3(kCells / kOneCells), dim3(kOneBlock), lds, st, hist, agg, sub_agg, occ_bits, work, bounds,
                               sub_bounds, sub_affine, cent, k, lab_table, masks, (uint8_t *)colour_labels, sub_table, sums, n_rows, flags, stats,
                               (uint16_t *)nullptr, 0u);
        if (tl.acc_out)
            hipLaunchKernelGGL((k_cube_pairs<uint8_t>), dim3(1), dim3(kBlock), 0, st, work, 1, occ_bits,
                               (const uint8_t *)colour_labels, sub_table, flags | kCubeNoEntries, sums, k, tl);
        return hipGetLastError();
    }
    static const uint32_t g_stage = env_grid("KMG_CUBE_GRID", 1536u), g_scan = env_grid("KMG_SCAN_GRID", kCubeGrid),
                          g_pairs = env_grid("KMG_PAIRS_GRID", kCubeGrid);
    CellWork *cw = (CellWork *)cell_work;
    if (!n_rows) n_rows = 1u;
    if (k <= 256u && tools_env_int(KMG_TOOLS_ENV("KMG_SPLIT_LONG"), 1) != 0) {
        flags |= kCubeSplitLong;
        hipError_t e = hipMemsetAsync(reinterpret_cast<uint32_t *>((CellWork *)cell_work + kCells) + kLongCount, 0, sizeof(uint32_t) * kLongSegs, st);
        if (e != hipSuccess) return e;
    }
#define KMG_CUBE(T, S)                                                                                                      \
    do {                                                                                                                    \
        hipLaunchKernelGGL((k_cube_stage<T, S>), dim3(g_stage), dim3(kBlock), lds_stage, st, agg, sub_agg, work, bounds,     \
                           sub_bounds, cent, k, masks, cw, (T *)colour_labels, sub_table, sums, n_rows, flags, stats);      \
        hipLaunchKernelGGL((k_cube_scan<T, S>), dim3(g_scan), dim3(kScanBlock), lds_scan, st, hist, sub_agg, work, cent, k,   \
                           lab_table, masks, cw, (T *)colour_labels, sub_table, sums, n_rows, repl, flags);                 \
        hipLaunchKernelGGL((k_cube_pairs<T>), dim3((flags & kCubeNoEntries) ? 1u : g_pairs), dim3(kBlock), 0, st, work,   \
                           S ? 1 : 0, occ_bits, (const T *)colour_labels, sub_table, flags, sums, k, tl);                   \
    } while (0)
    if (k <= 256) { if (with_sums) KMG_CUBE(uint8_t, true); else KMG_CUBE(uint8_t, false); }
    else          { if (with_sums) KMG_CUBE(uint16_t, true); else KMG_CUBE(uint16_t, false); }
#undef KMG_CUBE
    return hipGetLastError();
}

hipError_t launch_cube_entries(const uint32_t *work, const uint8_t *occ_bits, const void *colour_labels, uint16_t *sub_table,
                               uint32_t k, hipStream_t st)
{
    static const uint32_t g_pairs = env_grid("KMG_PAIRS_GRID", kCubeGrid);
    if (k <= 256)
        hipLaunchKernelGGL((k_cube_pairs<uint8_t>), dim3(g_pairs), dim3(kBlock), 0, st, work, work ? 1 : 0, occ_bits,
                           (const uint8_t *)colour_labels, sub_table, 0u, (int64_t *)nullptr, k, CubeTail());
    else
        hipLaunchKernelGGL((k_cube_pairs<uint16_t>), dim3(g_pairs), dim3(kBlock), 0, st, work, work ? 1 : 0, occ_bits,
                           (const uint16_t *)colour_labels, sub_table, 0u, (int64_t *)nullptr, k, CubeTail());
    return hipGetLastError();
}

}
```

### kmeans-gpu_amd/csrc/kmg_lloyd.hip

```cpp

#include <math.h>

#include "kmg_state.h"

static void drop_events(kmg_lloyd *s);
static void destroy_events(kmg_lloyd *s);
static int debug_refresh(kmg_lloyd *s, hipStream_t st, unsigned long long stage[8]);
static int side_flush(kmg_lloyd *s, hipStream_t st);
static void free_table(kmg_processor *p, ColourTable &t)
{
    block_give(p, t.blk, t.blk_cap);
    block_give(p, t.blk_alt, t.blk_alt_cap);
    block_give(p, t.blk_init, t.blk_init_cap);
    t = ColourTable();
}


static inline void *carve(void *base, size_t &off, size_t bytes)
{
    void *r = (uint8_t *)base + off;
    off += pad256(bytes);
    return r;
}

// ... 24 lines not shown
    const double one_launch = 4.85e-5 + 7.0e-8 * K, three_launches = 2.6e-5 + 2.0e-7 * K;
    if (!facts) return one_launch < three_launches ? one_launch : three_launches;
    return facts->hot ? three_launches : one_launch;
}

static bool table_pays(const kmg_processor *p, uint64_t n, uint32_t k, bool labels, const ImageFacts *facts)
{
    if (const int f = forced_strategy(p)) return f > 0;
    const double N = (double)n;
    const double N22 = (double)(1u << 22);
    const double label_pass = !labels ? 0.0 : (k > 256u ? N * 6.7e-12 : (N <= N22 ? 3.0e-6 + N * 4.4e-12 : 2.15e-5 + (N - N22) * 2.2e-12));
    const double table = cube_seconds(k, facts) + label_pass + (facts ? 0.0 : bind_seconds(n) / 16.0);
    const double scan = scan_seconds(n, k, facts ? facts->hot != 0u : true);
    return table < scan;
}

int ensure_bounds(kmg_processor *p, hipStream_t st)
{
    std::lock_guard<std::mutex> lock(p->mu);
    if (p->d_bounds) return KMG_OK;
    CellBounds *b = nullptr, *sb = nullptr;
    float4 *lab = nullptr;
    HIP_TRY(hipMalloc((void **)&b, sizeof(CellBounds) * kCells));
    hipError_t e = hipMalloc((void **)&sb, sizeof(CellBounds) * kSubCells);
    if (e == hipSuccess) e = hipMalloc((void **)&lab, sizeof(float4) << 24);
    if (e == hipSuccess) e = launch_cell_bounds(p->d_lut, b, sb, lab, st);
    if (e == hipSuccess) e = hipStreamSynchronize(st);
    if (e != hipSuccess) {
        (void)hipFree(b);
        if (sb) (void)hipFree(sb);
        if (lab) (void)hipFree(lab);
        return fail(e == hipErrorOutOfMemory ? KMG_ERR_OUT_OF_MEMORY : KMG_ERR_HIP, "colour tables failed: %s", hipGetErrorString(e));
    }
    p->d_lab_table = lab;
    p->d_sub_bounds = sb;
    p->d_bounds = b;
    return KMG_OK;
}

const float *affine_for(kmg_processor *p, uint32_t k, hipStream_t st)
{
    if (k > 256u) return nullptr;
    std::lock_guard<std::mutex> lock(p->mu);
    if (p->d_sub_affine || p->affine_failed || !p->d_lab_table) return p->d_sub_affine;
    float *a = nullptr;
    hipError_t e = hipMalloc((void **)&a, sub_affine_bytes());
    if (e == hipSuccess) e = launch_sub_affine(p->d_lab_table, p->d_sub_bounds, a, st);
    if (e == hipSuccess) e = hipStreamSynchronize(st);
    if (e != hipSuccess) {
        (void)hipGetLastError();
        if (a) (void)hipFree(a);
        p->affine_failed = true;
        return nullptr;
    }
    p->d_sub_affine = a;
    return a;
}

static int tables_from_histogram(kmg_lloyd *s, uint64_t n_pixels, hipStream_t st)
{
    ColourTable &t = s->tab;
    HIP_TRY(launch_cell_aggregates(t.d_hist, s->p->d_lab_table, t.d_agg, t.d_sub_agg, t.d_occ, st));
    HIP_TRY(launch_work_list(t.d_agg, t.d_work, s->k <= 256 ? n_pixels : 0, st));
    HIP_TRY(hipMemcpyAsync(&t.n_hot, t.d_work + kCells + 1, sizeof(uint32_t), hipMemcpyDeviceToHost, st));
    HIP_TRY(hipMemcpyAsync(&t.n_occ, t.d_work, sizeof(uint32_t), hipMemcpyDeviceToHost, st));
    HIP_TRY(hipStreamSynchronize(st));
    if (const char *e = KMG_TOOLS_ENV("KMG_HOT_CELLS")) { if (e[0] == '0') t.n_hot = 0; }
    t.d_work_share = nullptr;
    t.balance_work = nullptr;
    return KMG_OK;
}

static int bind_image_impl(kmg_lloyd *s, const uint8_t *d_rgba, uint64_t n, void *stream, bool want_tie, uint64_t first_index)
{
    if (!s || !d_rgba || n == 0) return fail(KMG_ERR_INVALID_ARGUMENT, "bad bind_image arguments");
    if (s->side) HIP_TRY(hipStreamSynchronize(s->side));
    s->lab_pending[0] = s->lab_pending[1] = false;
    if (n > 0xFFFFFFFFull) return fail(KMG_ERR_UNSUPPORTED, "image has more than 2^32-1 pixels");
    HIP_TRY(hipSetDevice(s->p->device));
    int rc;
    if ((rc = ensure_bounds(s->p, S(stream))) != KMG_OK) return rc;
    ColourTable &t = s->tab;
    if (!t.d_hist) {
        const size_t sizes[11] = {sizeof(uint32_t) << 24, sizeof(int64_t) * 4ull * kCells, sizeof(int64_t) * 4ull * kSubCells,
                                  (size_t)1 << 21, cube_work_bytes(), cube_masks_bytes(s->k),
                                  sizeof(uint32_t) * kWorkWords, (size_t)(s->k <= 256 ? 1 : 2) << 24, sub_table_bytes(),
                                  sizeof(uint32_t) * (kCells + 1), cube_balance_bytes()};
        size_t need = 0;
        for (size_t b : sizes) need += pad256(b);
        const hipError_t e = block_take(s->p, need, &t.blk, &t.blk_cap);
        if (e != hipSuccess) {
            t.blk = nullptr; t.blk_cap = 0;
            return fail(e == hipErrorOutOfMemory ? KMG_ERR_OUT_OF_MEMORY : KMG_ERR_HIP,
                        "colour table allocation failed: %s", hipGetErrorString(e));
        }
        size_t off = 0;
        t.d_hist = (uint32_t *)carve(t.blk, off, sizes[0]);
        t.d_agg = (int64_t *)carve(t.blk, off, sizes[1]);
        t.d_sub_agg = (int64_t *)carve(t.blk, off, sizes[2]);
        t.d_occ = (uint8_t *)carve(t.blk, off, sizes[3]);
        t.d_cell_work = carve(t.blk, off, sizes[4]);
        t.d_masks = (uint64_t *)carve(t.blk, off, sizes[5]);
        t.d_work = (uint32_t *)carve(t.blk, off, sizes[6]);
        t.d_colour_labels = carve(t.blk, off, sizes[7]);
        t.d_sub = (uint16_t *)carve(t.blk, off, sizes[8]);
        t.share_buf = (uint32_t *)carve(t.blk, off, sizes[9]);
        t.d_balance = (uint16_t *)carve(t.blk, off, sizes[10]);
    }
    t.d_work_share = nullptr;
    t.balance_work = nullptr;
    t.rgba = nullptr;
    t.tables_valid = false;
    t.tie_valid = false;
    t.bound_by_init = false;
    t.bound_by_caller = false;
    HIP_TRY(hipMemsetAsync(t.d_sub, 0xFF, sub_table_bytes(), S(stream)));
    if (t.d_sub_alt) HIP_TRY(hipMemsetAsync(t.d_sub_alt, 0xFF, sub_table_bytes(), S(stream)));
    if (n >= (1ull << 21)) {
        StreamBuf small, elems, keys;
        hipError_t e = small.alloc(s->p, sizeof(uint32_t) * (4 * 1024 + 1), S(stream));
        if (e == hipSuccess) e = elems.alloc(s->p, sizeof(uint16_t) * n, S(stream));
        if (e == hipSuccess && want_tie) e = keys.alloc(s->p, sizeof(uint32_t) * n, S(stream));
        if (e == hipSuccess)
            e = launch_partitioned_histogram((const uint32_t *)d_rgba, n, first_index, (uint32_t *)small.ptr, (uint16_t *)elems.ptr,
                                             (uint32_t *)keys.ptr, t.d_hist, t.d_tie, S(stream));
        if (e != hipSuccess)
            return fail(e == hipErrorOutOfMemory ? KMG_ERR_OUT_OF_MEMORY : KMG_ERR_HIP, "histogram failed: %s", hipGetErrorString(e));
    } else {
        HIP_TRY(hipMemsetAsync(t.d_hist, 0, sizeof(uint32_t) << 24, S(stream)));
        HIP_TRY(launch_histogram((const uint32_t *)d_rgba, n, t.d_hist, S(stream)));
        if (want_tie) {
            HIP_TRY(hipMemsetAsync(t.d_tie, 0, sizeof(uint32_t) << 24, S(stream)));
            HIP_TRY(launch_tie_keys((const uint32_t *)d_rgba, n, first_index, t.d_tie, S(stream)));
        }
    }
    if (want_tie) {
        t.tie_valid = true;
        t.tie_first = first_index;
    }
    int rc_agg;
    if ((rc_agg = tables_from_histogram(s, n, S(stream))) != KMG_OK) return rc_agg;
    if (want_tie) HIP_TRY(launch_init_records(t.d_work, s->p->d_bounds, t.d_init_cells, S(stream)));
    t.rgba = d_rgba;
    t.n = n;
    return KMG_OK;
}

extern "C" int kmg_lloyd_bind_image(kmg_lloyd *s, const uint8_t *d_rgba, uint64_t n, void *stream)
try {
    const int rc = bind_image_impl(s, d_rgba, n, stream, false, 0);
    if (rc == KMG_OK) s->tab.bound_by_caller = true;
    return rc;
}
KMG_ABI_CATCH

static int prepare_impl(kmg_lloyd *s, const uint8_t *d_rgba, uint64_t n, int want_labels, int *strategy, void *stream, bool caller)
{
    if (!s || !d_rgba || n == 0) return fail(KMG_ERR_INVALID_ARGUMENT, "bad prepare arguments");
    int chosen = 0;
    const bool fresh = s->tab.rgba == d_rgba && s->tab.n == n && s->tab.bound_by_init;
    s->tab.bound_by_init = false;
    const ImageFacts before = {s->tab.n_occ, s->tab.n_hot};
    bool try_table = n <= 0xFFFFFFFFull && table_pays(s->p, n, s->k, want_labels != 0, fresh ? &before : nullptr);
    if (try_table && !fresh && forced_strategy(s->p) == 0) {
        const ImageFacts dense = {kCells, 0u};
        const double N = (double)n, N22 = (double)(1u << 22);
        const double label_pass = !want_labels ? 0.0 : (s->k > 256u ? N * 6.7e-12 : (N <= N22 ? 3.0e-6 + N * 4.4e-12 : 2.15e-5 + (N - N22) * 2.2e-12));
        const bool sure = cube_seconds(s->k, &dense) + label_pass + bind_seconds(n) / 16.0 < scan_seconds(n, s->k, false);
        if (!sure) {
            uint32_t *d_probe = reinterpret_cast<uint32_t *>(s->d_nconv) + 1;
            uint32_t h[3] = {0u, 0u, 1u};
            HIP_TRY(launch_sparsity_probe((const uint32_t *)d_rgba, n, d_probe, S(stream)));
            HIP_TRY(hipMemcpyAsync(h, d_probe, sizeof h, hipMemcpyDeviceToHost, S(stream)));
            HIP_TRY(hipStreamSynchronize(S(stream)));
            double M = (double)h[0];
            for (int it = 0; it < 8 && h[0] < h[2]; ++it) M = (double)h[0] / (1.0 - exp(-(double)h[2] / (M > 1.0 ? M : 1.0)));
            const ImageFacts guess = {(uint32_t)(M < (double)kCells ? M : (double)kCells), h[1] * 10u >= h[2] ? 1u : 0u};
            const double table = cube_seconds(s->k, &guess) + label_pass + bind_seconds(n) / 16.0;
            try_table = table < scan_seconds(n, s->k, guess.hot != 0u);
            if (log_debug()) fprintf(stderr, "[kmeans_hip] prepare: %u of %u samples' cells, %u in crowded cells -> ~%u occupied%s: %s\n", h[0], h[2], h[1],
                                     guess.occupied, guess.hot ? ", hot" : "", try_table ? "bind" : "per-pixel scan");
        }
    }
    if (try_table) {
        if (!fresh) {
            int rc = bind_image_impl(s, d_rgba, n, stream, false, 0);
            if (rc != KMG_OK) return rc;
        }
        const ImageFacts facts = {s->tab.n_occ, s->tab.n_hot};
        if (fresh || table_pays(s->p, n, s->k, want_labels != 0, &facts)) {
            s->tab.bound_by_caller = caller;
            chosen = 1;
        } else {
// ... 75 lines not shown
    std::vector<uint32_t> hist(1u << 24);
    std::vector<uint16_t> labels(1u << 24);
    HIP_TRY(hipMemcpy(masks.data(), s->tab.d_masks, masks.size() * 8, hipMemcpyDeviceToHost));
    HIP_TRY(hipMemcpy(agg.data(), s->tab.d_agg, agg.size() * 8, hipMemcpyDeviceToHost));
    HIP_TRY(hipMemcpy(hist.data(), s->tab.d_hist, hist.size() * 4, hipMemcpyDeviceToHost));
    if (s->k <= 256) {
        std::vector<uint8_t> l8(1u << 24);
        HIP_TRY(hipMemcpy(l8.data(), s->tab.d_colour_labels, l8.size(), hipMemcpyDeviceToHost));
        for (size_t i = 0; i < l8.size(); ++i) labels[i] = l8[i];
    } else {
        HIP_TRY(hipMemcpy(labels.data(), s->tab.d_colour_labels, labels.size() * 2, hipMemcpyDeviceToHost));
    }
    for (int i = 0; i < 8; ++i) out[i] = 0;
    out[8] = stage[2]; out[9] = stage[3]; out[10] = stage[4]; out[11] = stage[5]; out[12] = stage[6]; out[13] = stage[7];
    for (uint32_t c = 0; c < kCells; ++c) {
        if (agg[4ull * c + 3] == 0) continue;
        uint64_t pop = 0;
        for (uint32_t w = 0; w < words; ++w) pop += (uint64_t)__builtin_popcountll(masks[(size_t)c * words + w]);
        out[0] += 1; out[1] += pop; out[2] += pop == 1; out[3] = std::max<uint64_t>(out[3], pop);
        int cell_first = -1;
        bool cell_one = true;
        for (uint32_t q = 0; q < 8; ++q) {
            int first = -1;
            bool one = true;
            for (uint32_t i = 0; i < 64; ++i) {
                const uint32_t col = c * kCellColours + q * 64 + i;
                if (!hist[col]) continue;
                if (first < 0) first = labels[col];
                one = one && first == (int)labels[col];
                if (cell_first < 0) cell_first = labels[col];
                cell_one = cell_one && cell_first == (int)labels[col];
            }
            out[5] += first >= 0;
            out[6] += first >= 0 && one;
        }
        out[4] += cell_one;
    }
    for (uint32_t v : hist) out[7] += v != 0;
    return KMG_OK;
}
KMG_ABI_CATCH

extern "C" int kmg_debug_check_pairs(kmg_lloyd *s, uint64_t out[3], void *stream)
try {
    if (!s || !out) return fail(KMG_ERR_INVALID_ARGUMENT, "bad check_pairs arguments");
    if (!s->tab.rgba || !s->tab.tables_valid) return fail(KMG_ERR_INVALID_ARGUMENT, "no current colour table");
    if (s->k > 256) return fail(KMG_ERR_INVALID_ARGUMENT, "pair entries exist for k <= 256 only");
    HIP_TRY(hipSetDevice(s->p->device));
    HIP_TRY(hipStreamSynchronize(S(stream)));
    int rc_;
    if ((rc_ = debug_refresh(s, S(stream), nullptr)) != KMG_OK) return rc_;
    std::vector<uint32_t> hist(1u << 24), pairs(kCells);
    std::vector<uint8_t> labels(1u << 24);
    HIP_TRY(hipMemcpy(hist.data(), s->tab.d_hist, hist.size() * 4, hipMemcpyDeviceToHost));
    HIP_TRY(hipMemcpy(labels.data(), s->tab.d_colour_labels, labels.size(), hipMemcpyDeviceToHost));
    HIP_TRY(hipMemcpy(pairs.data(), reinterpret_cast<const uint32_t *>(s->tab.d_sub + kSubCells + kCells),
                      pairs.size() * 4, hipMemcpyDeviceToHost));
    std::vector<uint32_t> hot(1 + kHotMax, 0u);
    if (s->tab.n_hot) HIP_TRY(hipMemcpy(hot.data(), s->tab.d_work + kCells + 1, sizeof(uint32_t) * (1 + kHotMax), hipMemcpyDeviceToHost));
    std::vector<uint8_t> in_lds(kCells, 0);
    for (uint32_t h = 0; h < s->tab.n_hot && h < kHotMax; ++h) {
        const uint32_t e = pairs[hot[1 + h]];
        const bool one_label = (e & 0xFFu) == ((e >> 8) & 0xFFu) && (e >> 23) == 0u;
        if (!one_label) in_lds[hot[1 + h]] = 1;
    }
    out[0] = out[1] = out[2] = 0;
    for (uint32_t c = 0; c < (1u << 24); ++c) {
        if (!hist[c]) continue;
        if (in_lds[c >> 9]) { out[1] += hist[c]; out[2] += hist[c]; continue; }
        uint32_t r, g, b;
        index_to_rgb(c, r, g, b);
        const uint32_t e = pairs[c >> 9];
        const uint32_t px = r | (g << 8) | (b << 16);
        const uint32_t got = pair_decode(e, pair_project(pair_dir_word((e >> 16) & 127u), px));
        out[2] += hist[c];
        if (got == kPairFine) continue;
        out[1] += hist[c];
        out[0] += got != labels[c];
    }
    return KMG_OK;
}
KMG_ABI_CATCH

static CubeBalance next_balance(ColourTable &t, const uint32_t *work)
{
    if (t.balance_work != work) { t.balance_work = work; t.balance_pass = 0; }
    CubeBalance b;
    b.state = t.d_balance;
    b.pass = t.balance_pass++;
    return b;
}

static int debug_refresh(kmg_lloyd *s, hipStream_t st, unsigned long long stage[8] = nullptr)
{
    ColourTable &t = s->tab;
    int rc_;
    if (t.d_work_share) return fail(KMG_ERR_INVALID_ARGUMENT, "statistics / checks of a bound image need the whole cube: a cell share is set");
    if ((rc_ = side_flush(s, st)) != KMG_OK) return rc_;
    unsigned long long *d_stage = reinterpret_cast<unsigned long long *>(s->d_partials) + 4ull * s->k;
    HIP_TRY(hipMemsetAsync(s->d_partials, 0, sizeof(int64_t) * (4ull * s->k + 8ull), st));
    HIP_TRY(launch_cube(t.d_hist, t.d_agg, t.d_sub_agg, t.d_occ, t.d_work, s->p->d_bounds, s->p->d_sub_bounds, s->d_cent, s->k,
                        s->p->d_lab_table, t.d_masks, t.d_cell_work, t.d_colour_labels, t.d_sub, s->d_partials, 1u, 1u | (t.n_hot ? kCubeHot : 0u), d_stage, st,
                        nullptr, affine_for(s->p, s->k, st)));
    t.entries_valid = true;
    if (stage) HIP_TRY(hipMemcpyAsync(stage, d_stage, 8 * sizeof(unsigned long long), hipMemcpyDeviceToHost, st));
    HIP_TRY(hipStreamSynchronize(st));
    return KMG_OK;
}

static int side_flush(kmg_lloyd *s, hipStream_t st)
{
    for (int i = 0; i < 2; ++i)
        if (s->lab_pending[i]) {
            HIP_TRY(hipStreamWaitEvent(st, s->ev_lab[i], 0));
            s->lab_pending[i] = false;
        }
    return KMG_OK;
}

static bool table_bound(const kmg_lloyd *s, const uint8_t *d_rgba, uint64_t n)
{
    return s->tab.rgba != nullptr && s->tab.rgba == d_rgba && s->tab.n == n;
}

static int ensure_entries(kmg_lloyd *s, hipStream_t st)
{
    ColourTable &t = s->tab;
    if (t.entries_valid) return KMG_OK;
    HIP_TRY(launch_cube_entries(t.d_work_share ? t.d_work_share : t.d_work, t.d_occ, t.d_colour_labels, t.d_sub, s->k, st));
    t.entries_valid = true;
    return KMG_OK;
}

static int table_assign(kmg_lloyd *s, const uint8_t *d_rgba, uint64_t n, uint32_t *d_labels, int64_t *d_sums,
                        uint32_t rows, hipStream_t st, bool update_after = false, bool defer_entries = false, bool add_in_place = false)
{
    if (d_labels) defer_entries = false;
    ColourTable &t = s->tab;
    if (add_in_place) {
        if (d_labels || update_after || rows != 1u) return fail(KMG_ERR_INVALID_ARGUMENT, "table_assign: in-place sums are sums only");
        t.bound_by_init = false;
        int rc2;
        if ((rc2 = side_flush(s, st)) != KMG_OK) return rc2;
        const CubeBalance bal = next_balance(t, t.d_work_share ? t.d_work_share : t.d_work);
        PROF_LAUNCH(s, KMG_K_CUBE, st, launch_cube(t.d_hist, t.d_agg, t.d_sub_agg, t.d_occ, t.d_work_share ? t.d_work_share : t.d_work,
                                                   s->p->d_bounds, s->p->d_sub_bounds, s->d_cent, s->k, s->p->d_lab_table, t.d_masks, t.d_cell_work,
                                                   t.d_colour_labels, t.d_sub, d_sums, 1u, t.n_hot ? kCubeHot : 0u, nullptr, st, nullptr,
                                                   affine_for(s->p, s->k, st), &bal));
        t.entries_valid = true;
        t.tables_valid = t.d_work_share == nullptr;
        return KMG_OK;
    }
    if (t.d_work_share && (d_labels || update_after || rows != 1u))
        return fail(KMG_ERR_INVALID_ARGUMENT, "a cell share is set: this pass returns one share's sums only -- no label map, no "
                    "update, no partial rows (all-reduce the sums, all-gather the tables, then kmg_lloyd_labels_from_tables)");
    t.bound_by_init = false;
    int rc_;
    if ((rc_ = side_flush(s, st)) != KMG_OK) return rc_;
    if (rows == 1u) {
        if (s->acc_int_dirty) HIP_TRY(hipMemsetAsync(s->d_acc_int, 0, sizeof(int64_t) * 4ull * s->k, st));
        s->acc_int_dirty = true;
        CubeTail tail;
        tail.acc_out = d_sums;
        tail.do_update = update_after ? 1 : 0;
        tail.convergence = s->p->opt.convergence;
        tail.cent = s->d_cent;
        tail.n_converged = s->d_nconv;
        static const bool tail_rides = tools_env_int(KMG_TOOLS_ENV("KMG_TAIL_ON_LABELS"), 1) != 0;
        const bool tail_on_labels = tail_rides && d_labels != nullptr && s->k <= 256u && cube_single_launch(s->k, t.n_hot ? kCubeHot : 0u);
        const CubeBalance bal = next_balance(t, t.d_work_share ? t.d_work_share : t.d_work);
        PROF_LAUNCH(s, KMG_K_CUBE, st, launch_cube(t.d_hist, t.d_agg, t.d_sub_agg, t.d_occ, t.d_work_share ? t.d_work_share : t.d_work,
                                                   s->p->d_bounds, s->p->d_sub_bounds,
                                                   s->d_cent, s->k, s->p->d_lab_table, t.d_masks, t.d_cell_work, t.d_colour_labels, t.d_sub,
                                                   s->d_acc_int, 1u, (defer_entries ? kCubeNoEntries : 0u) | (t.n_hot ? kCubeHot : 0u), nullptr, st,
                                                   tail_on_labels ? nullptr : &tail, affine_for(s->p, s->k, st), &bal));
        t.entries_valid = !defer_entries;
        if (tail_on_labels) {
            t.tables_valid = true;
            PROF_LAUNCH(s, KMG_K_LABELS, st, launch_labels((const uint32_t *)d_rgba, n, t.d_colour_labels, t.d_sub, s->k, nullptr, d_labels, st,
                                                           s->reserve_cus, t.n_hot ? t.d_work + kCells + 1 : nullptr, &tail, s->d_acc_int));
            s->acc_int_dirty = false;
            if (update_after) t.tables_valid = false;
            return KMG_OK;
        }
        s->acc_int_dirty = false;
    } else {
        if (update_after) return fail(KMG_ERR_INVALID_ARGUMENT, "table_assign: update_after needs the final sums");
        HIP_TRY(hipMemsetAsync(d_sums, 0, sizeof(int64_t) * 4ull * s->k * rows, st));
        PROF_LAUNCH(s, KMG_K_CUBE, st, launch_cube(t.d_hist, t.d_agg, t.d_sub_agg, t.d_occ, t.d_work, s->p->d_bounds, s->p->d_sub_bounds,
                                                   s->d_cent, s->k, s->p->d_lab_table, t.d_masks, t.d_cell_work, t.d_colour_labels, t.d_sub,
                                                   d_sums, rows, t.n_hot ? kCubeHot : 0u, nullptr, st, nullptr, affine_for(s->p, s->k, st)));
        t.entries_valid = true;
    }
    t.tables_valid = t.d_work_share == nullptr;
    if (d_labels)
        PROF_LAUNCH(s, KMG_K_LABELS, st, launch_labels((const uint32_t *)d_rgba, n, t.d_colour_labels, t.d_sub, s->k, nullptr, d_labels, st, s->reserve_cus, t.n_hot ? t.d_work + kCells + 1 : nullptr));
    if (update_after) t.tables_valid = false;
    return KMG_OK;
}

int lloyd_create_impl(kmg_processor *p, uint32_t k, kmg_lloyd **out, hipStream_t pool_stream)
{
    if (!p || !out) return fail(KMG_ERR_INVALID_ARGUMENT, "bad lloyd_create arguments");
    *out = nullptr;
    if (k == 0) return fail(KMG_ERR_INVALID_ARGUMENT, "k must be an integer higher than 0");
    if (k > KMG_MAX_K) return fail(KMG_ERR_UNSUPPORTED, "k = %u exceeds KMG_MAX_K = %u", k, KMG_MAX_K);
    HIP_TRY(hipSetDevice(p->device));
    kmg_lloyd *s = new (std::nothrow) kmg_lloyd();
    if (!s) return fail(KMG_ERR_OUT_OF_MEMORY, "host allocation failed");
    s->p = p;
    s->k = k;
    s->d_cent = nullptr; s->d_partials = nullptr; s->d_acc = nullptr; s->d_nconv = nullptr;
    s->d_key = nullptr; s->d_dist = nullptr; s->dist_cap = 0; s->last_rows = 0; s->prof = 0; s->init_colours = false;
    s->side = nullptr; s->ev_cube = nullptr; s->ev_lab[0] = s->ev_lab[1] = nullptr;
    s->lab_pending[0] = s->lab_pending[1] = false; s->set = 0;
    s->pooled = pool_stream != nullptr;
    s->pool_stream = pool_stream;
    s->ws = nullptr; s->ws_cap = 0; s->dist_blk_cap = 0;
    s->h_slot = host_slot_take(p);
    const size_t sizes[6] = {sizeof(Centroid) * k, sizeof(int64_t) * 4ull * k * 2048ull, sizeof(int64_t) * 4ull * k, sizeof(uint32_t),
                             sizeof(unsigned long long), sizeof(int64_t) * 4ull * k};
    size_t need = 0;
    for (size_t b : sizes) need += pad256(b);
    hipError_t e = block_take(p, need, &s->ws, &s->ws_cap);
    if (e == hipSuccess) {
        size_t off = 0;
        s->d_cent = (Centroid *)carve(s->ws, off, sizes[0]);
        s->d_partials = (int64_t *)carve(s->ws, off, sizes[1]);
        s->d_acc = (int64_t *)carve(s->ws, off, sizes[2]);
        s->d_nconv = (uint32_t *)carve(s->ws, off, sizes[3]);
        s->d_key = (unsigned long long *)carve(s->ws, off, sizes[4]);
        s->d_acc_int = (int64_t *)carve(s->ws, off, sizes[5]);
        s->acc_int_dirty = true;
        auto zero = [&](void *ptr, size_t bytes) {
            return s->pooled ? hipMemsetAsync(ptr, 0, bytes, pool_stream) : hipMemset(ptr, 0, bytes);
        };
        e = zero(s->d_cent, sizeof(Centroid) * k);
        if (e == hipSuccess) e = zero(s->d_nconv, sizeof(uint32_t));
    } else {
        s->ws = nullptr; s->ws_cap = 0;
    }
    if (e != hipSuccess) {
        kmg_lloyd_destroy(s);
        return fail(e == hipErrorOutOfMemory ? KMG_ERR_OUT_OF_MEMORY : KMG_ERR_HIP,
                    "lloyd workspace allocation failed: %s", hipGetErrorString(e));
    }
    *out = s;
    return KMG_OK;
}

extern "C" int kmg_lloyd_create(kmg_processor *p, uint32_t k, kmg_lloyd **out)
try {
    return lloyd_create_impl(p, k, out, nullptr);
}
KMG_ABI_CATCH

extern "C" void kmg_lloyd_destroy(kmg_lloyd *s)
try {
    if (!s) return;
    (void)hipSetDevice(s->p->device);
    if (s->side) {
        (void)hipStreamSynchronize(s->side);
        (void)hipStreamDestroy(s->side);
        (void)hipEventDestroy(s->ev_cube); (void)hipEventDestroy(s->ev_lab[0]); (void)hipEventDestroy(s->ev_lab[1]);
    }
    if (s->pooled) (void)hipStreamSynchronize(s->pool_stream); else (void)hipDeviceSynchronize();
    block_give(s->p, s->ws, s->ws_cap);
    block_give(s->p, s->d_dist, s->dist_blk_cap);
    free_table(s->p, s->tab);
    destroy_events(s);
    host_slot_give(s->p, s->h_slot);
    delete s;
}
KMG_ABI_CATCH_VOID

extern "C" int kmg_lloyd_set_centroids(kmg_lloyd *s, const float *c4, void *stream)
try {
    if (!s || !c4) return fail(KMG_ERR_INVALID_ARGUMENT, "bad set_centroids arguments");
    HIP_TRY(hipSetDevice(s->p->device));
    std::vector<Centroid> h(s->k);
    for (uint32_t i = 0; i < s->k; ++i) {
        h[i].L = c4[4 * i]; h[i].a = c4[4 * i + 1]; h[i].b = c4[4 * i + 2];
        h[i].C = chroma(h[i].a, h[i].b);
    }
    s->tab.tables_valid = false;
    s->tab.bound_by_init = false;
    HIP_TRY(hipMemcpyAsync(s->d_cent, h.data(), sizeof(Centroid) * s->k, hipMemcpyHostToDevice, S(stream)));
    HIP_TRY(hipStreamSynchronize(S(stream)));
    return KMG_OK;
}
KMG_ABI_CATCH

extern "C" int kmg_lloyd_get_centroids(kmg_lloyd *s, float *c4, void *stream)
try {
    if (!s || !c4) return fail(KMG_ERR_INVALID_ARGUMENT, "bad get_centroids arguments");
    HIP_TRY(hipSetDevice(s->p->device));
    std::vector<Centroid> own;
    Centroid *h = static_cast<Centroid *>(s->h_slot);
    if (!h || sizeof(Centroid) * s->k > kHostSlotBytes) { own.resize(s->k); h = own.data(); }
    HIP_TRY(hipMemcpyAsync(h, s->d_cent, sizeof(Centroid) * s->k, hipMemcpyDeviceToHost, S(stream)));
    HIP_TRY(hipStreamSynchronize(S(stream)));
    for (uint32_t i = 0; i < s->k; ++i) {
        c4[4 * i] = h[i].L; c4[4 * i + 1] = h[i].a; c4[4 * i + 2] = h[i].b; c4[4 * i + 3] = 1.0f;
    }
    return KMG_OK;
}
KMG_ABI_CATCH

static bool init_table_pays(const kmg_processor *p, uint64_t n, uint32_t k)
{
    if (const int f = forced_strategy(p)) return f > 0;
    const double N = (double)n, passes = (double)(k - 1);
    const double pixels = k >= 32u ? (0.3 * k + 18.0) * (9.0e-6 + N * 30.0e-12) : passes * (8.0e-6 + N * 7.0e-12);
    const double colours = passes * 0.9e-5 + (passes < 16.0 ? passes : 16.0) * 3.0e-5 +
                           (n >= (1ull << 21) ? 1.5 * bind_seconds(n) : 5.0e-5 + N * 2.0e-10);
    return colours < pixels;
}

static int init_over_colours(kmg_lloyd *s, const uint8_t *d_rgba, uint64_t n, uint64_t first_index, bool *colours,
                             void *stream)
{
    *colours = false;
    if (first_index + n > 0xFFFFFFF0ull || !init_table_pays(s->p, n, s->k)) {
        if (s->tab.rgba == d_rgba) s->tab.rgba = nullptr;
        return KMG_OK;
    }
    ColourTable &t = s->tab;
    if (!t.d_tie) {
        const size_t need = pad256(sizeof(uint32_t) << 24) + pad256(sizeof(float) << 24) + pad256(init_scratch_bytes());
        const hipError_t e = block_take(s->p, need, &t.blk_init, &t.blk_init_cap);
        if (e != hipSuccess) {
            t.blk_init = nullptr; t.blk_init_cap = 0;
            return fail(e == hipErrorOutOfMemory ? KMG_ERR_OUT_OF_MEMORY : KMG_ERR_HIP, "init tables allocation failed: %s", hipGetErrorString(e));
        }
        size_t off = 0;
        t.d_tie = (uint32_t *)carve(t.blk_init, off, sizeof(uint32_t) << 24);
        t.d_cdist = (float *)carve(t.blk_init, off, sizeof(float) << 24);
        t.d_init_cells = carve(t.blk_init, off, init_scratch_bytes());
    }
    int rc;
    if ((rc = bind_image_impl(s, d_rgba, n, stream, true, first_index)) != KMG_OK) return rc;
    t.bound_by_init = true;
    *colours = true;
    return KMG_OK;
}

extern "C" int kmg_lloyd_init_centroids(kmg_lloyd *s, const uint8_t *d_rgba, uint32_t w, uint32_t h, void *stream)
try {
    if (!s || !d_rgba || !w || !h) return fail(KMG_ERR_INVALID_ARGUMENT, "bad init_centroids arguments");
    HIP_TRY(hipSetDevice(s->p->device));
    const uint64_t n = (uint64_t)w * h;
    if (n > 0xFFFFFFFFull) return fail(KMG_ERR_UNSUPPORTED, "image has more than 2^32-1 pixels");
    s->tab.tables_valid = false;
    const int32_t x0 = (int32_t)((float)w * 0.5625f);
    const int32_t y0 = (int32_t)((float)h * 0.93359375f);
    const uint64_t i0 = (uint64_t)y0 * w + (uint64_t)x0;
    const uint32_t *rgba = (const uint32_t *)d_rgba;
    HIP_TRY(launch_init_first(rgba, i0, s->p->d_lut, s->d_cent, s->d_key, S(stream)));
    if (s->k == 1 && s->tab.rgba == d_rgba) s->tab.rgba = nullptr;
    if (s->k > 1) {
        int rc;
        bool colours = false;
        if ((rc = init_over_colours(s, d_rgba, n, 0, &colours, stream)) != KMG_OK) return rc;
        if (!colours && s->dist_cap < n) {
            if (s->d_dist) {
                HIP_TRY(hipStreamSynchronize(S(stream)));
                HIP_TRY(hipFree(s->d_dist));
                s->d_dist = nullptr; s->dist_cap = 0; s->dist_blk_cap = 0;
// ... 338 lines not shown
    drop_events(s);
    return KMG_OK;
}
KMG_ABI_CATCH

extern "C" int kmg_lloyd_update(kmg_lloyd *s, const int64_t *d_acc4, void *stream)
try {
    if (!s || !d_acc4) return fail(KMG_ERR_INVALID_ARGUMENT, "bad update arguments");
    HIP_TRY(hipSetDevice(s->p->device));
    s->tab.tables_valid = false;
    PROF_LAUNCH(s, KMG_K_UPDATE, S(stream), launch_update(d_acc4, s->k, s->p->opt.convergence, s->d_cent, s->d_nconv, S(stream)));
    return KMG_OK;
}
KMG_ABI_CATCH

static int assign_update_impl(kmg_lloyd *s, const uint8_t *d_rgba, uint64_t n, uint32_t *d_labels, int64_t *d_acc4,
                              int do_update, void *stream, bool defer_entries)
{
    if (!s || !d_rgba || n == 0 || !d_acc4) return fail(KMG_ERR_INVALID_ARGUMENT, "bad assign_update arguments");
    HIP_TRY(hipSetDevice(s->p->device));
    if (table_bound(s, d_rgba, n)) return table_assign(s, d_rgba, n, d_labels, d_acc4, 1u, S(stream), do_update != 0, defer_entries);
    int rc;
    if ((rc = assign_pass(s, d_rgba, n, d_labels, true, S(stream))) != KMG_OK) return rc;
    if (reduce_update_fits(s->last_rows, s->k)) {
        if (do_update) s->tab.tables_valid = false;
        PROF_LAUNCH(s, KMG_K_REDUCE, S(stream), launch_reduce_update(s->d_partials, s->last_rows, s->k, d_acc4, do_update, s->p->opt.convergence,
                                                                    s->d_cent, s->d_nconv, S(stream)));
        return KMG_OK;
    }
    PROF_LAUNCH(s, KMG_K_REDUCE, S(stream), launch_reduce_partials(s->d_partials, s->last_rows, s->k, d_acc4, S(stream)));
    return do_update ? kmg_lloyd_update(s, d_acc4, stream) : KMG_OK;
}

extern "C" int kmg_lloyd_assign_update(kmg_lloyd *s, const uint8_t *d_rgba, uint64_t n, uint32_t *d_labels, int64_t *d_acc4,
                                       int do_update, void *stream)
try {
    return assign_update_impl(s, d_rgba, n, d_labels, d_acc4, do_update, stream, false);
}
KMG_ABI_CATCH

extern "C" int kmg_lloyd_iterate(kmg_lloyd *s, const uint8_t *d_rgba, uint64_t n, uint32_t *d_labels, int64_t *d_acc4,
                                 int update_first, void *stream)
try {
    if (!s || !d_rgba || n == 0 || !d_acc4) return fail(KMG_ERR_INVALID_ARGUMENT, "bad iterate arguments");
    HIP_TRY(hipSetDevice(s->p->device));
    int rc;
    if (!table_bound(s, d_rgba, n) || !d_labels) {
        if (update_first && (rc = kmg_lloyd_update(s, d_acc4, stream)) != KMG_OK) return rc;
        return kmg_lloyd_assign_accumulate(s, d_rgba, n, d_labels, d_acc4, stream);
    }
    hipStream_t st = S(stream);
    ColourTable &t = s->tab;
    if (t.d_work_share) return fail(KMG_ERR_INVALID_ARGUMENT, "iterate: a cell share is set (kmg_lloyd_set_cell_share)");
    if (!s->side) {
        int least = 0, greatest = 0;
        HIP_TRY(hipDeviceGetStreamPriorityRange(&least, &greatest));
        HIP_TRY(hipStreamCreateWithPriority(&s->side, hipStreamNonBlocking, greatest));
        HIP_TRY(hipEventCreateWithFlags(&s->ev_cube, hipEventDisableTiming));
        HIP_TRY(hipEventCreateWithFlags(&s->ev_lab[0], hipEventDisableTiming));
        HIP_TRY(hipEventCreateWithFlags(&s->ev_lab[1], hipEventDisableTiming));
    }
    const size_t sub_bytes = sub_table_bytes();
    if (!t.d_colour_labels_alt) {
        const size_t lab_bytes = (size_t)(s->k <= 256 ? 1 : 2) << 24;
        HIP_TRY(block_take(s->p, pad256(lab_bytes) + pad256(sub_bytes), &t.blk_alt, &t.blk_alt_cap));
        size_t off = 0;
        t.d_colour_labels_alt = carve(t.blk_alt, off, lab_bytes);
        t.d_sub_alt = (uint16_t *)carve(t.blk_alt, off, sub_bytes);
        HIP_TRY(hipMemsetAsync(t.d_sub_alt, 0xFF, sub_bytes, st));
    }
    std::swap(t.d_colour_labels, t.d_colour_labels_alt);
    std::swap(t.d_sub, t.d_sub_alt);
    s->set ^= 1;
    t.tables_valid = false;
    t.bound_by_init = false;
    auto issue = [&]() -> int {
        if (s->lab_pending[s->set]) {
            HIP_TRY(hipStreamWaitEvent(st, s->ev_lab[s->set], 0));
            s->lab_pending[s->set] = false;
        }
        if (update_first)
            PROF_LAUNCH(s, KMG_K_UPDATE, st, launch_update(d_acc4, s->k, s->p->opt.convergence, s->d_cent, s->d_nconv, st));
        HIP_TRY(hipMemsetAsync(d_acc4, 0, sizeof(int64_t) * 4ull * s->k, st));
        const CubeBalance bal = next_balance(t, t.d_work);
        PROF_LAUNCH(s, KMG_K_CUBE, st, launch_cube(t.d_hist, t.d_agg, t.d_sub_agg, t.d_occ, t.d_work, s->p->d_bounds, s->p->d_sub_bounds,
                                                   s->d_cent, s->k, s->p->d_lab_table, t.d_masks, t.d_cell_work, t.d_colour_labels, t.d_sub,
                                                   d_acc4, 1u, t.n_hot ? kCubeHot : 0u, nullptr, st, nullptr, affine_for(s->p, s->k, st), &bal));
        return KMG_OK;
    };
    if ((rc = issue()) != KMG_OK) {
        std::swap(t.d_colour_labels, t.d_colour_labels_alt);
        std::swap(t.d_sub, t.d_sub_alt);
        s->set ^= 1;
        return rc;
    }
    t.tables_valid = true;
    t.entries_valid = true;
    HIP_TRY(hipEventRecord(s->ev_cube, st));
    HIP_TRY(hipStreamWaitEvent(s->side, s->ev_cube, 0));
    PROF_LAUNCH(s, KMG_K_LABELS, s->side, launch_labels((const uint32_t *)d_rgba, n, t.d_colour_labels, t.d_sub, s->k, nullptr,
                                                        d_labels, s->side, s->reserve_cus, t.n_hot ? t.d_work + kCells + 1 : nullptr));
    HIP_TRY(hipEventRecord(s->ev_lab[s->set], s->side));
    s->lab_pending[s->set] = true;
    return KMG_OK;
}
KMG_ABI_CATCH

extern "C" int kmg_lloyd_flush(kmg_lloyd *s, void *stream)
try {
    if (!s) return fail(KMG_ERR_INVALID_ARGUMENT, "bad flush arguments");
    HIP_TRY(hipSetDevice(s->p->device));
    return side_flush(s, S(stream));
}
KMG_ABI_CATCH

extern "C" int kmg_lloyd_converged_count(kmg_lloyd *s, uint32_t *count, void *stream)
try {
    if (!s || !count) return fail(KMG_ERR_INVALID_ARGUMENT, "bad converged_count arguments");
    HIP_TRY(hipSetDevice(s->p->device));
    if (s->h_slot) {
        HIP_TRY(hipMemcpyAsync(s->h_slot, s->d_nconv, sizeof(uint32_t), hipMemcpyDeviceToHost, S(stream)));
        HIP_TRY(hipStreamSynchronize(S(stream)));
        *count = *static_cast<const volatile uint32_t *>(s->h_slot);
        return KMG_OK;
    }
    HIP_TRY(hipMemcpyAsync(count, s->d_nconv, sizeof(uint32_t), hipMemcpyDeviceToHost, S(stream)));
    HIP_TRY(hipStreamSynchronize(S(stream)));
    return KMG_OK;
}
KMG_ABI_CATCH

extern "C" int kmg_lloyd_run(kmg_lloyd *s, const uint8_t *d_rgba, uint64_t n, uint32_t *d_labels,
                             uint32_t *iterations, void *stream)
try {
    if (!s || !d_rgba || n == 0) return fail(KMG_ERR_INVALID_ARGUMENT, "bad lloyd_run arguments");
    if (s->tab.d_work_share && table_bound(s, d_rgba, n))
        return fail(KMG_ERR_INVALID_ARGUMENT, "lloyd_run: a cell share is set (kmg_lloyd_set_cell_share): the loop would update from one share's sums");
    const kmg_options &o = s->p->opt;
    int rc;
    const bool callers = table_bound(s, d_rgba, n) && s->tab.bound_by_caller;
    if (!callers)
        if ((rc = prepare_impl(s, d_rgba, n, 0, nullptr, stream, false)) != KMG_OK) return rc;
    const bool table = table_bound(s, d_rgba, n);
    uint32_t *loop_labels = table ? nullptr : d_labels;
    auto checked = [&](uint32_t it) { return it > 0 && it % o.check_period == 0; };
    if (!table && assign_loop_fits(n) && assign_loop_scratch_bytes(s->k) <= sizeof(int64_t) * 4ull * s->k * 2048ull) {
        hipStream_t st = S(stream);
        if ((rc = side_flush(s, st)) != KMG_OK) return rc;
        int64_t *acc3[3] = {s->d_partials, s->d_partials + 4ull * s->k, s->d_partials + 8ull * s->k};
        Centroid *cur = s->d_cent, *alt = reinterpret_cast<Centroid *>(s->d_partials + 12ull * s->k);
        HIP_TRY(hipMemsetAsync(s->d_partials, 0, sizeof(int64_t) * 12ull * s->k, st));
        const uint32_t *px = (const uint32_t *)d_rgba;
        s->tab.tables_valid = false;
        PROF_LAUNCH(s, KMG_K_ASSIGN, st, launch_assign_loop(px, n, cur, alt, s->k, s->p->d_lut, d_labels, nullptr, acc3[0], acc3[1], 0,
                                                          o.convergence, s->d_nconv, st));
        uint32_t it = 0;
        for (it = 0; it < o.max_iterations; ++it) {
            const uint32_t l = it + 1u;
            PROF_LAUNCH(s, KMG_K_ASSIGN, st, launch_assign_loop(px, n, cur, alt, s->k, s->p->d_lut, d_labels, acc3[(l + 2u) % 3u], acc3[l % 3u],
                                                              acc3[(l + 1u) % 3u], 1, o.convergence, s->d_nconv, st));
            std::swap(cur, alt);
            if (checked(it)) {
                uint32_t conv = 0;
                if ((rc = kmg_lloyd_converged_count(s, &conv, stream)) != KMG_OK) return rc;
                if (conv >= s->k) {
                    if (log_debug()) fprintf(stderr, "[kmeans_hip] We have convergence, checked at iteration %u\n", it);
                    break;
                }
            }
        }
// ... 39 lines not shown
```

### kmeans-gpu_amd/csrc/kmg_state.h

```cpp
#pragma once

#include <hip/hip_runtime.h>

#include <stdarg.h>
#include <stdio.h>
#include <stdlib.h>
#include <string.h>

#include <algorithm>
#include <atomic>
#include <chrono>
#include <exception>
#include <mutex>
#include <thread>
#include <new>
#include <vector>

#include "kmg_color.h"
#include "kmg_internal.h"
#include "kmg_kernels.h"
#include "kmg_octree.h"
#include "kmg_table.h"

using namespace kmg;

#define HIP_TRY(expr)                                                                          \
    do {                                                                                       \
        hipError_t e_ = (expr);                                                                \
        if (e_ != hipSuccess)                                                                  \
            return fail(e_ == hipErrorOutOfMemory ? KMG_ERR_OUT_OF_MEMORY : KMG_ERR_HIP,       \
                        "%s failed: %s (%s:%d)", #expr, hipGetErrorString(e_), __FILE__, __LINE__); \
    } while (0)

#define PROF_LAUNCH(s_, id_, st_, expr)                                                        \
    do {                                                                                       \
        if ((s_)->prof & (1u << (id_))) {                                                      \
            ProfEvent pe_; pe_.id = (id_);                                                     \
            if ((s_)->pool.size() >= 2) {                                                      \
                pe_.e0 = (s_)->pool.back(); (s_)->pool.pop_back();                             \
                pe_.e1 = (s_)->pool.back(); (s_)->pool.pop_back();                             \
            } else {                                                                           \
                HIP_TRY(hipEventCreate(&pe_.e0)); HIP_TRY(hipEventCreate(&pe_.e1));            \
            }                                                                                  \
            HIP_TRY(hipEventRecord(pe_.e0, (st_)));                                            \
            HIP_TRY(expr);                                                                     \
            HIP_TRY(hipEventRecord(pe_.e1, (st_)));                                            \
            (s_)->events.push_back(pe_);                                                       \
        } else {                                                                               \
            HIP_TRY(expr);                                                                     \
        }                                                                                      \
    } while (0)

struct kmg_processor {
    int device;
    kmg_options opt;
    std::atomic<int> strategy{0};
    std::atomic<uint32_t> alpha_cutoff{0};
    float *d_lut;
    std::mutex mu;
    CellBounds *d_bounds;
    CellBounds *d_sub_bounds;
    float4 *d_lab_table;
    float *d_sub_affine;
    bool affine_failed;
    std::vector<hipStream_t> idle_streams;
    std::vector<std::pair<void *, size_t>> idle_arenas;
    uint64_t n_block_malloc = 0, n_block_reuse = 0;
    hipMemPool_t pool;
    void *h_page = nullptr;
    bool h_page_tried = false;
    std::vector<uint16_t> h_free;
};

constexpr size_t kHostPageBytes = (size_t)1 << 20, kHostSlotBytes = 8192;

void *host_slot_take(kmg_processor *p);
void host_slot_give(kmg_processor *p, void *slot);
hipError_t block_take(kmg_processor *p, size_t bytes, void **ptr, size_t *cap);
void block_give(kmg_processor *p, void *ptr, size_t cap);

static inline size_t pad256(size_t bytes) { return (bytes + 255u) & ~(size_t)255u; }

struct ProfEvent { int id; hipEvent_t e0, e1; };

struct ColourTable {
    const uint8_t *rgba = nullptr;
    uint64_t n = 0;
    uint32_t *d_hist = nullptr;
    int64_t *d_agg = nullptr;
    int64_t *d_sub_agg = nullptr;
    uint8_t *d_occ = nullptr;
    void *d_cell_work = nullptr;
    uint64_t *d_masks = nullptr;
    uint32_t *d_work = nullptr;
    uint32_t n_hot = 0;
    uint32_t n_occ = 0;
    uint16_t *d_balance = nullptr;
    const uint32_t *balance_work = nullptr;
    uint32_t balance_pass = 0;
    uint32_t *share_buf = nullptr;
    uint32_t *d_work_share = nullptr;
    bool tables_valid = false;
    bool entries_valid = false;
    void *d_colour_labels = nullptr;
    uint16_t *d_sub = nullptr;
    void *d_colour_labels_alt = nullptr;
    uint16_t *d_sub_alt = nullptr;
    uint32_t *d_tie = nullptr;
    float *d_cdist = nullptr;
    void *d_init_cells = nullptr;
    bool tie_valid = false;
    bool bound_by_init = false;
    bool bound_by_caller = false;
    uint64_t tie_first = 0;
    void *blk = nullptr, *blk_alt = nullptr, *blk_init = nullptr;
    size_t blk_cap = 0, blk_alt_cap = 0, blk_init_cap = 0;
};

struct kmg_lloyd {
    kmg_processor *p;
    uint32_t k;
    Centroid *d_cent;
    int64_t *d_partials;
    int64_t *d_acc;
    int64_t *d_acc_int;
    bool acc_int_dirty;
    uint32_t *d_nconv;
    void *h_slot = nullptr;
    unsigned long long *d_key;
    float *d_dist;
    uint64_t dist_cap;
    size_t dist_blk_cap;
    void *ws;
    size_t ws_cap;
    uint32_t last_rows;
    bool init_colours;
    uint32_t reserve_cus = 0;
    bool pooled;
    hipStream_t pool_stream;
    ColourTable tab;
    hipStream_t side;
    hipEvent_t ev_cube;
    hipEvent_t ev_lab[2];
    bool lab_pending[2];
    int set;
    uint32_t prof;
    std::vector<ProfEvent> events;
    std::vector<hipEvent_t> pool;
};

static inline hipStream_t S(void *s) { return (hipStream_t)s; }

static inline int forced_strategy(const kmg_processor *p)
{
    if (const char *e = KMG_TOOLS_ENV("KMG_STRATEGY")) {
        if (!strcmp(e, "brute")) return -1;
        if (!strcmp(e, "table")) return 1;
    }
    const int st = p->strategy.load(std::memory_order_relaxed) & 3;
    return st == KMG_STRATEGY_TABLE ? 1 : (st == KMG_STRATEGY_SCAN ? -1 : 0);
}

namespace {
struct DevBuf {
    void *ptr = nullptr;
    ~DevBuf() { if (ptr) (void)hipFree(ptr); }
    hipError_t alloc(size_t bytes) { return hipMalloc(&ptr, bytes); }
};

static hipError_t pool_alloc(kmg_processor *p, void **ptr, size_t bytes, hipStream_t stream)
{
    return p->pool ? hipMallocFromPoolAsync(ptr, bytes, p->pool, stream) : hipMallocAsync(ptr, bytes, stream);
}

struct StreamBuf {
    void *ptr = nullptr;
    hipStream_t st = nullptr;
    ~StreamBuf() { if (ptr) (void)hipFreeAsync(ptr, st); }
    hipError_t alloc(kmg_processor *p, size_t bytes, hipStream_t stream) { st = stream; return pool_alloc(p, &ptr, bytes, stream); }
};

struct ArenaGuard {
// ... 45 lines not shown
```

### kmeans-gpu_amd/csrc/kmg_table.h

```cpp
#pragma once

#include <hip/hip_runtime.h>
#include <stdint.h>

#include "kmg_kernels.h"

namespace kmg {

constexpr uint32_t kCells = 32768;
constexpr uint32_t kCellColours = 512;
constexpr uint32_t kSubCells = kCells * 8;
constexpr uint32_t kCubeGrid = 2048;
constexpr uint32_t kMergeRows = 64;
constexpr uint32_t kHotMax = 56;
constexpr uint32_t kWorkWords = kCells + 1 + 1 + kHotMax;

constexpr uint16_t kSubEmpty = 0xFFFF;
constexpr uint16_t kSubMixed = 0xFFFE;

struct alignas(16) CellBounds {
    float L0, L1, a0, a1, b0, b1, C0, C1, wC0, wC1, wH0, wH1;
    float pad[4];
};

// ... 21 lines not shown
}

inline uint32_t mask_words(uint32_t k) { return (k + 63u) / 64u; }
inline size_t cube_masks_bytes(uint32_t k)
{
    return sizeof(uint64_t) * ((size_t)kCells * mask_words(k) + (k <= 256 ? (size_t)kCells * 8u * 4u : 0u));
}

constexpr uint32_t kPairDirs = 125;
constexpr uint32_t kPairFine = 0xFFFFFFFFu;

__host__ __device__ inline uint32_t pair_dir_code(int nx, int ny, int nz)
{
    return (uint32_t)((nx + 2) * 25 + (ny + 2) * 5 + (nz + 2));
}

__host__ __device__ inline uint32_t pair_dir_word(uint32_t code)
{
    const int nx = (int)(code / 25u) - 2, ny = (int)((code / 5u) % 5u) - 2, nz = (int)(code % 5u) - 2;
    const int bias = 7 * ((nx < 0 ? -nx : 0) + (ny < 0 ? -ny : 0) + (nz < 0 ? -nz : 0));
    return ((uint32_t)nx & 255u) | (((uint32_t)ny & 255u) << 8) | (((uint32_t)nz & 255u) << 16) | ((uint32_t)bias << 24);
}

__host__ __device__ inline uint32_t pair_entry(uint32_t A, uint32_t B, uint32_t code, uint32_t tlo, uint32_t w)
{
    return (A & 255u) | ((B & 255u) << 8) | (code << 16) | (tlo << 23) | (w << 29);
}

__host__ __device__ inline int pair_project(uint32_t dir_word, uint32_t px)
{
    return (int)(int8_t)(dir_word & 255u) * (int)(px & 7u) + (int)(int8_t)((dir_word >> 8) & 255u) * (int)((px >> 8) & 7u) +
           (int)(int8_t)((dir_word >> 16) & 255u) * (int)((px >> 16) & 7u) + (int)(dir_word >> 24);
}

__host__ __device__ inline uint32_t pair_decode(uint32_t e, int p)
{
    const int tlo = (int)((e >> 23) & 63u);
    const int w = (int)(e >> 29);
    const int thr = tlo + w + (w == 7 ? 64 : 0);
    if (p < tlo) return e & 255u;
    if (p >= thr) return (e >> 8) & 255u;
    return kPairFine;
}

hipError_t launch_cell_bounds(const float *lut, CellBounds *bounds, CellBounds *sub_bounds, float4 *lab_table, hipStream_t st);
hipError_t launch_histogram(const uint32_t *rgba, uint64_t n, uint32_t *hist, hipStream_t st);
hipError_t launch_partitioned_histogram(const uint32_t *rgba, uint64_t n, uint64_t first_index, uint32_t *small,
                                        uint16_t *elems, uint32_t *keys, uint32_t *hist, uint32_t *tie, hipStream_t st);
hipError_t launch_cell_aggregates(const uint32_t *hist, const float4 *lab_table, int64_t *agg, int64_t *sub_agg, uint8_t *occ_bits,
                                  hipStream_t st);
hipError_t launch_work_list(const int64_t *agg, uint32_t *work, uint64_t n_pixels, hipStream_t st);
hipError_t launch_sparsity_probe(const uint32_t *rgba, uint64_t n, uint32_t *out3, hipStream_t st);
hipError_t launch_work_share(const uint32_t *work, uint32_t part, uint32_t parts, uint32_t *out, hipStream_t st);
hipError_t launch_tie_keys(const uint32_t *rgba, uint64_t n, uint64_t first_index, uint32_t *tie, hipStream_t st);
size_t init_scratch_bytes();
hipError_t launch_init_records(const uint32_t *work, const CellBounds *bounds, void *init_scratch, hipStream_t st);
hipError_t launch_init_pass_cells(const uint32_t *tie, const uint8_t *occ_bits, const float4 *lab_table, Centroid *cent,
                                  uint32_t j, int do_pass, float *dist, void *init_scratch, unsigned long long *band_key,
                                  const uint32_t *pick_rgba, const float *lut, hipStream_t st);
hipError_t launch_init_cells_multi(const uint32_t *tie, const uint8_t *occ_bits, const float4 *lab_table, Centroid *cent, uint32_t k,
                                   uint32_t launch, float *dist, void *init_scratch, const uint32_t *pick_rgba, const float *lut,
                                   hipStream_t st);
const uint32_t *init_cells_multi_count(const void *init_scratch, uint32_t launch);
size_t cube_work_bytes();
constexpr uint32_t kCubeNoEntries = 0x10000u;
constexpr uint32_t kCubeHot = 0x40000u;
constexpr uint32_t kCubeSplitLong = 0x80000u;
constexpr uint32_t kCubeSmallMaxK = 32;
bool cube_single_launch(uint32_t k, uint32_t flags);
hipError_t launch_cube_entries(const uint32_t *work, const uint8_t *occ_bits, const void *colour_labels, uint16_t *sub_table,
                               uint32_t k, hipStream_t st);
struct CubeTail {
    int64_t *acc_out = nullptr;
    int do_update = 0;
    float convergence = 0.0f;
    Centroid *cent = nullptr;
    uint32_t *n_converged = nullptr;
};
struct CubeBalance {
    uint16_t *state = nullptr;
    uint32_t pass = 0;
};
size_t cube_balance_bytes();
hipError_t launch_cube(const uint32_t *hist, const int64_t *agg, const int64_t *sub_agg, const uint8_t *occ_bits,
                       const uint32_t *work, const CellBounds *bounds, const CellBounds *sub_bounds, const Centroid *cent,
                       uint32_t k, const float4 *lab_table, uint64_t *masks, void *cell_work, void *colour_labels,
                       uint16_t *sub_table, int64_t *sums, uint32_t n_rows, uint32_t flags, unsigned long long *stats,
                       hipStream_t st, const CubeTail *tail = nullptr, const float *sub_affine = nullptr,
                       const CubeBalance *balance = nullptr);
size_t sub_affine_bytes();
hipError_t launch_sub_affine(const float4 *lab_table, const CellBounds *sub_bounds, float *affine, hipStream_t st);
hipError_t launch_labels(const uint32_t *rgba, uint64_t n, const void *colour_labels,
                         const uint16_t *sub_table, uint32_t k, const uint32_t *pal, uint32_t *labels,
                         hipStream_t st, uint32_t reserve_cus = 0, const uint32_t *hot = nullptr,
                         const CubeTail *tail = nullptr, int64_t *tail_sums = nullptr);

hipError_t launch_offset_candidates(const CellBounds *bounds, const Centroid *cent, uint32_t k, float threshold,
                                    uint64_t *masks, hipStream_t st);
hipError_t launch_dither_pruned(const uint32_t *rgba, uint32_t w, uint32_t rows, uint32_t row0, const Centroid *cent,
                                uint32_t k, const float *lut, const uint32_t *pal, float threshold,
                                const uint64_t *masks, uint32_t *out, hipStream_t st);

constexpr uint32_t kListBytes = 32, kListMax = 2 * kListBytes - 1;
constexpr uint32_t kLabCells = 40u * 72u * 72u;
constexpr size_t kLabListBytes = 2ull * kLabCells * kListBytes;
constexpr uint32_t kLabListMaxK = 512;
size_t lab_list_bytes(uint32_t k);
hipError_t launch_lab_candidates(const Centroid *cent, uint32_t k, float threshold, bool two_closest, uint8_t *lists, hipStream_t st);
hipError_t launch_meld_lists(const uint32_t *rgba, uint64_t n, const Centroid *cent, uint32_t k, const float *lut,
                             const uint8_t *lists, uint32_t *out, hipStream_t st);
hipError_t launch_check_lab_lists_two(const Centroid *cent, uint32_t k, const uint8_t *lists, const float *lut,
                                      unsigned long long *violations, hipStream_t st);
hipError_t launch_dither_lists(const uint32_t *rgba, uint32_t w, uint32_t rows, uint32_t row0, const Centroid *cent, uint32_t k,
                               const float *lut, const uint32_t *pal, float threshold, const uint8_t *lists, uint32_t *out,
                               hipStream_t st);
hipError_t launch_check_lab_lists(const Centroid *cent, uint32_t k, const uint8_t *lists, const float *lut, float threshold,
                                  unsigned long long *violations, hipStream_t st);
hipError_t launch_check_offset_masks(const Centroid *cent, uint32_t k, const uint64_t *masks, const float *lut,
                                     float threshold, unsigned long long *violations, hipStream_t st);

hipError_t launch_meld_candidates(const CellBounds *bounds, const Centroid *cent, uint32_t k, uint64_t *masks, hipStream_t st);
hipError_t launch_check_meld_masks(const Centroid *cent, uint32_t k, const uint64_t *masks, const float *lut,
                                   unsigned long long *violations, hipStream_t st);

hipError_t launch_check_bounds(const CellBounds *bounds, const CellBounds *sub_bounds, const Centroid *cent, uint32_t k,
                               const uint64_t *masks, const void *colour_labels, const float *lut,
                               unsigned long long *violations, hipStream_t st);

}
```

Measured before the change: 308.8 billion pixels/s.

## Remember per-cell pair slab direction across passes and try neighbour directions

Adds a per-cell byte buffer, double-buffered by pass, that records which slab direction won when building the two-label pair entry. On the next pass the builder also tries the remembered direction and a couple of rotating neighbours, and keeps whichever leaves the fewest unresolved colours. The aim is narrower or better-resolved pair entries, so fewer pixels fall back to a slow per-pixel path in the label and accumulate kernels. In exchange the entry build runs several slab evaluations with wave reductions per pending cell and adds extra byte reads and writes per cell.

```diff
diff --git a/kmeans-gpu_amd/csrc/kmg_cube.hip b/kmeans-gpu_amd/csrc/kmg_cube.hip
--- a/kmeans-gpu_amd/csrc/kmg_cube.hip
+++ b/kmeans-gpu_amd/csrc/kmg_cube.hip
@@ -56,7 +56,64 @@
 
 
 
-__device__ __forceinline__ uint32_t cell_pair_entry(const uint32_t idx[8], uint32_t occ, uint32_t lane)
+struct PairCell {
+    uint32_t labA, labB;
+    uint32_t occ, rest, notB;
+    uint32_t n_occ;
+};
+
+struct PairSlab {
+    int tlo, thi;
+    bool low_side;
+    uint32_t unresolved;
+};
+
+__device__ __forceinline__ PairSlab pair_slab(const PairCell &c, int nx, int ny, int nz, uint32_t lane, bool count)
+{
+    const int xl = (int)(((lane >> 5) & 1u) * 4u + ((lane >> 1) & 3u));
+    const int yl = (int)(((lane >> 4) & 1u) * 4u + (lane & 1u) * 2u);
+    const int zl = (int)(((lane >> 3) & 1u) * 4u);
+    const int bias = 7 * ((nx < 0 ? -nx : 0) + (ny < 0 ? -ny : 0) + (nz < 0 ? -nz : 0));
+    const int p0 = nx * xl + ny * yl + nz * zl + bias;
+    int p[8];
+#pragma unroll
+    for (int q = 0; q < 8; ++q) p[q] = p0 + ny * (q >> 2) + nz * (q & 3);
+    uint32_t tl = 63u, hi = 64u;
+#pragma unroll
+    for (int q = 0; q < 8; ++q) {
+        if ((c.rest >> q) & 1u) tl = min(tl, (uint32_t)p[q]);
+        if ((c.notB >> q) & 1u) hi = min(hi, (uint32_t)(63 - p[q]));
+    }
+    u16x2 packed = __builtin_bit_cast(u16x2, tl | (hi << 16));
+    packed = __builtin_elementwise_min(packed, __builtin_bit_cast(u16x2, dpp_u32<kDppXor1>(__builtin_bit_cast(uint32_t, packed))));
+    packed = __builtin_elementwise_min(packed, __builtin_bit_cast(u16x2, dpp_u32<kDppXor2>(__builtin_bit_cast(uint32_t, packed))));
+    packed = __builtin_elementwise_min(packed, __builtin_bit_cast(u16x2, dpp_u32<kDppHalfMirror>(__builtin_bit_cast(uint32_t, packed))));
+    packed = __builtin_elementwise_min(packed, __builtin_bit_cast(u16x2, dpp_u32<kDppMirror>(__builtin_bit_cast(uint32_t, packed))));
+    packed = __builtin_elementwise_min(packed, __builtin_bit_cast(u16x2, (uint32_t)__builtin_amdgcn_update_dpp(-1, (int)__builtin_bit_cast(uint32_t, packed), 0x142, 0xA, 0xF, false)));
+    packed = __builtin_elementwise_min(packed, __builtin_bit_cast(u16x2, (uint32_t)__builtin_amdgcn_update_dpp(-1, (int)__builtin_bit_cast(uint32_t, packed), 0x143, 0xC, 0xF, false)));
+    const uint32_t pk = lane_value(__builtin_bit_cast(uint32_t, packed), 63);
+    PairSlab s;
+    s.tlo = (int)(pk & 0xFFFFu);
+    s.thi = 63 - (int)(pk >> 16);
+    s.low_side = true;
+    s.unresolved = 0u;
+    const bool wide = s.thi + 1 - s.tlo > 6;
+    if (count || wide) {
+        uint32_t low = 0, high = 0;
+#pragma unroll
+        for (int q = 0; q < 8; ++q) {
+            if ((c.occ >> q) & 1u) { low += p[q] < s.tlo ? 1u : 0u; high += p[q] > s.thi ? 1u : 0u; }
+        }
+        const uint32_t lh = wave_add_u32(low | (high << 10));
+        s.low_side = (lh & 1023u) >= (lh >> 10);
+        s.unresolved = c.n_occ - (wide ? max(lh & 1023u, lh >> 10) : (lh & 1023u) + (lh >> 10));
+    }
+    return s;
+}
+
+template <uint32_t NEIGHBOURS = kPairNeighbours>
+__device__ __forceinline__ uint32_t cell_pair_entry(const uint32_t idx[8], uint32_t occ, uint32_t lane, uint32_t prev_code,
+                                                    uint32_t dir_step, uint32_t *winner)
 {
     uint32_t rem = occ;
     uint32_t lab0 = 0, lab1 = 0, lab2 = 0, cnt0 = 0, cnt1 = 0, cnt2 = 0, msk0 = 0, msk1 = 0, msk2 = 0, n_occ = 0;
@@ -86,14 +143,19 @@
     uint32_t b = a == 0u ? 1u : 0u;
     if (a != 1u && b != 1u && cnt1 > sel3(b, cnt0, cnt1, cnt2)) b = 1;
     if (a != 2u && cnt2 > sel3(b, cnt0, cnt1, cnt2)) b = 2;
-    const uint32_t labA = sel3(a, lab0, lab1, lab2), labB = sel3(b, lab0, lab1, lab2);
+    PairCell c;
+    c.labA = sel3(a, lab0, lab1, lab2); c.labB = sel3(b, lab0, lab1, lab2);
     const uint32_t mA = sel3(a, msk0, msk1, msk2), mB = sel3(b, msk0, msk1, msk2);
-    const uint32_t rest = occ & ~mA;
+    c.occ = occ;
+    c.rest = occ & ~mA;
+    c.notB = occ & ~mB;
+    c.n_occ = n_occ;
     const uint32_t nA = sel3(a, cnt0, cnt1, cnt2), nR = n_occ - nA;
-    if (nR == 0u) return pair_entry(labA, labA, 0u, 0u, 0u);
+    *winner = kPairNoMemory;
+    if (nR == 0u) return pair_entry(c.labA, c.labA, 0u, 0u, 0u);
 
     const uint32_t half = ((lane >> 5) & 1u) | (((lane >> 4) & 1u) << 10) | (((lane >> 3) & 1u) << 20);
-    const uint32_t hR = wave_add_u32((uint32_t)__builtin_popcount(rest) * half);
+    const uint32_t hR = wave_add_u32((uint32_t)__builtin_popcount(c.rest) * half);
     const uint32_t hA = wave_add_u32((uint32_t)__builtin_popcount(mA) * half);
     const int gx = (int)((hR & 1023u) * nA) - (int)((hA & 1023u) * nR);
     const int gy = (int)(((hR >> 10) & 1023u) * nA) - (int)(((hA >> 10) & 1023u) * nR);
@@ -102,44 +164,41 @@
     const int m = ax > ay ? (ax > az ? ax : az) : (ay > az ? ay : az);
     int nx = 2, ny = 0, nz = 0;
     if (m > 0) { nx = round_dir(gx, m); ny = round_dir(gy, m); nz = round_dir(gz, m); }
-
-    const int xl = (int)(((lane >> 5) & 1u) * 4u + ((lane >> 1) & 3u));
-    const int yl = (int)(((lane >> 4) & 1u) * 4u + (lane & 1u) * 2u);
-    const int zl = (int)(((lane >> 3) & 1u) * 4u);
-    const int bias = 7 * ((nx < 0 ? -nx : 0) + (ny < 0 ? -ny : 0) + (nz < 0 ? -nz : 0));
-    const int p0 = nx * xl + ny * yl + nz * zl + bias;
-    int p[8];
-#pragma unroll
-    for (int q = 0; q < 8; ++q) p[q] = p0 + ny * (q >> 2) + nz * (q & 3);
-    const uint32_t notB = occ & ~mB;
-    uint32_t tl = 63u, hi = 64u;
-#pragma unroll
-    for (int q = 0; q < 8; ++q) {
-        if ((rest >> q) & 1u) tl = min(tl, (uint32_t)p[q]);
-        if ((notB >> q) & 1u) hi = min(hi, (uint32_t)(63 - p[q]));
-    }
-    u16x2 packed = __builtin_bit_cast(u16x2, tl | (hi << 16));
-    packed = __builtin_elementwise_min(packed, __builtin_bit_cast(u16x2, dpp_u32<kDppXor1>(__builtin_bit_cast(uint32_t, packed))));
-    packed = __builtin_elementwise_min(packed, __builtin_bit_cast(u16x2, dpp_u32<kDppXor2>(__builtin_bit_cast(uint32_t, packed))));
-    packed = __builtin_elementwise_min(packed, __builtin_bit_cast(u16x2, dpp_u32<kDppHalfMirror>(__builtin_bit_cast(uint32_t, packed))));
-    packed = __builtin_elementwise_min(packed, __builtin_bit_cast(u16x2, dpp_u32<kDppMirror>(__builtin_bit_cast(uint32_t, packed))));
-    packed = __builtin_elementwise_min(packed, __builtin_bit_cast(u16x2, (uint32_t)__builtin_amdgcn_update_dpp(-1, (int)__builtin_bit_cast(uint32_t, packed), 0x142, 0xA, 0xF, false)));
-    packed = __builtin_elementwise_min(packed, __builtin_bit_cast(u16x2, (uint32_t)__builtin_amdgcn_update_dpp(-1, (int)__builtin_bit_cast(uint32_t, packed), 0x143, 0xC, 0xF, false)));
-    const uint32_t pk = lane_value(__builtin_bit_cast(uint32_t, packed), 63);
-    const int tlo = (int)(pk & 0xFFFFu);
-    const int thi = 63 - (int)(pk >> 16);
+    const uint32_t hcode = pair_dir_code(nx, ny, nz);
+
+    const bool memory = NEIGHBOURS != kPairHeuristicOnly && prev_code < kPairDirs;
+    const uint32_t n_try = memory ? 2u + NEIGHBOURS : 1u;
+    uint32_t best_key = 0xFFFFFFFFu, best_slab = 0u;
+#pragma unroll 1
+    for (uint32_t t = 0; t < n_try; ++t) {
+        uint32_t ccode = hcode;
+        if (t) {
+            int cx = (int)(prev_code / 25u) - 2, cy = (int)((prev_code / 5u) % 5u) - 2, cz = (int)(prev_code % 5u) - 2;
+            if (t > 1u) {
+                const uint32_t j = (dir_step + t - 2u) % 6u;
+                const int d = (j & 1u) ? -1 : 1;
+                if ((j >> 1) == 0u) cx += d; else if ((j >> 1) == 1u) cy += d; else cz += d;
+            }
+            const int big = max(max(cx < 0 ? -cx : cx, cy < 0 ? -cy : cy), cz < 0 ? -cz : cz);
+            ccode = pair_dir_code(cx, cy, cz);
+            if (big == 0 || big > 2 || ccode == hcode) continue;
+        }
+        const PairSlab sc = pair_slab(c, (int)(ccode / 25u) - 2, (int)((ccode / 5u) % 5u) - 2, (int)(ccode % 5u) - 2, lane, memory);
+        const uint32_t key = (sc.unresolved << 8) | (t ? ccode + 1u : 0u);
+        if (key < best_key) {
+            best_key = key;
+            best_slab = (uint32_t)sc.tlo | ((uint32_t)(sc.thi + 1) << 6) | (sc.low_side ? 1u << 13 : 0u);
+        }
+    }
+    const uint32_t code = (best_key & 255u) ? (best_key & 255u) - 1u : hcode;
+    nx = (int)(code / 25u) - 2; ny = (int)((code / 5u) % 5u) - 2; nz = (int)(code % 5u) - 2;
+    const int tlo = (int)(best_slab & 63u), thi = (int)((best_slab >> 6) & 127u) - 1;
+    *winner = code;
     const int w = thi + 1 > tlo ? thi + 1 - tlo : 0;
-    const uint32_t code = pair_dir_code(nx, ny, nz);
-    if (w <= 6) return pair_entry(labA, labB, code, (uint32_t)tlo, (uint32_t)w);
-    uint32_t low = 0, high = 0;
-#pragma unroll
-    for (int q = 0; q < 8; ++q) {
-        if ((occ >> q) & 1u) { low += p[q] < tlo ? 1u : 0u; high += p[q] > thi ? 1u : 0u; }
-    }
-    const uint32_t lh = wave_add_u32(low | (high << 10));
-    if ((lh & 1023u) >= (lh >> 10)) return pair_entry(labA, labB, code, (uint32_t)tlo, 7u);
+    if (w <= 6) return pair_entry(c.labA, c.labB, code, (uint32_t)tlo, (uint32_t)w);
+    if ((best_slab >> 13) & 1u) return pair_entry(c.labA, c.labB, code, (uint32_t)tlo, 7u);
     const int range = 7 * ((nx < 0 ? -nx : nx) + (ny < 0 ? -ny : ny) + (nz < 0 ? -nz : nz));
-    return pair_entry(labB, labA, pair_dir_code(-nx, -ny, -nz), (uint32_t)(range - thi), 7u);
+    return pair_entry(c.labB, c.labA, pair_dir_code(-nx, -ny, -nz), (uint32_t)(range - thi), 7u);
 }
 
 __device__ __forceinline__ uint32_t merge_state(uint32_t a, uint32_t b)
@@ -171,6 +230,17 @@
 static_assert(sizeof(CellWork) == 128, "CellWork layout");
 
 constexpr uint32_t kPairPending = 0xFFFFFFFEu;
+
+struct DirMemory {
+    const uint8_t *prev = nullptr;
+    uint8_t *next = nullptr;
+    uint32_t step = 0;
+};
+
+__device__ __forceinline__ uint32_t remembered_direction(const DirMemory &dm, uint32_t cell)
+{
+    return dm.prev ? __builtin_amdgcn_readfirstlane((uint32_t)dm.prev[cell]) : kPairNoMemory;
+}
 
 constexpr uint32_t kLongSegs = 16, kLongSegCap = kCells / kLongSegs, kLongCount = 0, kLongCells = 64;
 constexpr size_t kListsWords = kLongCells + kCells;
@@ -821,7 +891,7 @@
                                                        const uint8_t *__restrict__ occ_bits,
                                                        const LabelT *__restrict__ colour_labels,
                                                        uint16_t *__restrict__ sub_table, uint32_t flags,
-                                                       int64_t *__restrict__ sums, uint32_t k, CubeTail tail)
+                                                       int64_t *__restrict__ sums, uint32_t k, CubeTail tail, DirMemory dirs)
 {
     if (tail.acc_out && blockIdx.x == gridDim.x - 1u) {
         __shared__ uint32_t s_count;
@@ -840,14 +910,21 @@
         const uint32_t cell = cells ? __builtin_amdgcn_readfirstlane(cells[wi]) : wi;
         if (sizeof(LabelT) == 1) {
             uint32_t *pair_entry_ptr = reinterpret_cast<uint32_t *>(sub_table + kSubCells + kCells) + cell;
-            if (__builtin_amdgcn_readfirstlane(*pair_entry_ptr) != kPairPending) continue;
+            if (__builtin_amdgcn_readfirstlane(*pair_entry_ptr) != kPairPending) {
+                if (dirs.next && lane == 0u) dirs.next[cell] = (uint8_t)kPairNoMemory;
+                continue;
+            }
             const uint2 lv = *reinterpret_cast<const uint2 *>(colour_labels + (uint64_t)cell * kCellColours + lane * 8u);
             const uint32_t occ = occ_bits ? (uint32_t)occ_bits[(uint64_t)cell * 64u + lane] : 0xFFu;
             uint32_t idx[8];
 #pragma unroll
             for (uint32_t q = 0; q < 4u; ++q) { idx[q] = (lv.x >> (8u * q)) & 0xFFu; idx[4u + q] = (lv.y >> (8u * q)) & 0xFFu; }
-            const uint32_t e = cell_pair_entry(idx, occ, lane);
-            if (lane == 0u) *pair_entry_ptr = e;
+            uint32_t won;
+            const uint32_t e = cell_pair_entry(idx, occ, lane, remembered_direction(dirs, cell), dirs.step, &won);
+            if (lane == 0u) {
+                *pair_entry_ptr = e;
+                if (dirs.next) dirs.next[cell] = (uint8_t)won;
+            }
         } else {
             uint32_t st = lane < 8u ? (uint32_t)sub_table[cell * 8u + lane] : (uint32_t)kSubEmpty;
 #pragma unroll
@@ -949,7 +1026,7 @@
                                                             uint8_t *__restrict__ colour_labels,
                                                             uint16_t *__restrict__ sub_table,
                                                             int64_t *__restrict__ sums, uint32_t n_rows, uint32_t flags,
-                                                            unsigned long long *__restrict__ stats)
+                                                            unsigned long long *__restrict__ stats, DirMemory dirs)
 {
     extern __shared__ float4 smem4[];
     float4 *s_cent = smem4;
@@ -1093,7 +1170,10 @@
             const uint32_t x4 = (decided ? X : 0u) * 0x01010101u;
             const uint4 xv = make_uint4(x4, x4, x4, x4);
             if (uniform) {
-                if (sub == 0u) pair_entries[cell] = pair_entry(xmin, xmin, 0u, 0u, 0u);
+                if (sub == 0u) {
+                    pair_entries[cell] = pair_entry(xmin, xmin, 0u, 0u, 0u);
+                    if (dirs.next) dirs.next[cell] = (uint8_t)kPairNoMemory;
+                }
                 if (flags & 1u) {
                     const uint32_t m4 = xmin * 0x01010101u;
                     uint4 *dst = reinterpret_cast<uint4 *>(colour_labels + (uint64_t)cell * kCellColours + sub * 64u);
@@ -1305,7 +1385,9 @@
                 uint32_t idx[8];
 #pragma unroll
                 for (uint32_t q = 0; q < 4u; ++q) { idx[q] = (lv.x >> (8u * q)) & 0xFFu; idx[4u + q] = (lv.y >> (8u * q)) & 0xFFu; }
-                e = cell_pair_entry(idx, occ, lane);
+                uint32_t won;
+                e = cell_pair_entry(idx, occ, lane, remembered_direction(dirs, pcell), dirs.step, &won);
+                if (dirs.next && lane == 0u) dirs.next[pcell] = (uint8_t)won;
             }
             if (lane == 0u) pair_entries[pcell] = e;
             *reinterpret_cast<uint2 *>(colour_labels + (uint64_t)pcell * kCellColours + lane * 8u) = lv;
@@ -1364,7 +1446,7 @@
     const CellBounds *__restrict__ sub_bounds, const float *__restrict__ sub_affine, const Centroid *__restrict__ cent, uint32_t k,
     const float4 *__restrict__ lab_table, uint64_t *__restrict__ masks_out, uint8_t *__restrict__ colour_labels,
     uint16_t *__restrict__ sub_table, int64_t *__restrict__ sums, uint32_t n_rows, uint32_t flags,
-    unsigned long long *__restrict__ stats, uint16_t *__restrict__ bal_state, uint32_t bal_pass)
+    unsigned long long *__restrict__ stats, uint16_t *__restrict__ bal_state, uint32_t bal_pass, DirMemory dirs)
 {
     extern __shared__ float4 smem4[];
     float4 *s_cent = smem4;
@@ -1610,7 +1692,10 @@
             const uint32_t x4 = (settled ? X : 0u) * 0x01010101u;
             const uint4 xv = make_uint4(x4, x4, x4, x4);
             if (uniform) {
-                if (sub == 0u) pair_entries[cell] = pair_entry(Xu, Xu, 0u, 0u, 0u);
+                if (sub == 0u) {
+                    pair_entries[cell] = pair_entry(Xu, Xu, 0u, 0u, 0u);
+                    if (dirs.next) dirs.next[cell] = (uint8_t)kPairNoMemory;
+                }
                 if (flags & 1u) {
                     const uint32_t m4 = Xu * 0x01010101u;
                     uint4 *dst = reinterpret_cast<uint4 *>(colour_labels + (uint64_t)cell * kCellColours + sub * 64u);
@@ -1669,7 +1754,7 @@
         const uint32_t n_items = s_count[0];
         KMG_STAMP_VALUE(8, n_items); KMG_STAMP_VALUE(10, s_count[8]);
 
-        auto cell_entry = [&](const uint32_t ps) {
+        auto cell_entry = [&](const uint32_t ps) __attribute__((always_inline)) {
             const uint32_t pcell = __builtin_amdgcn_readfirstlane(s_cell[ps]);
             const uint2 lv = *reinterpret_cast<const uint2 *>(s_lbl + ps * kCellColours + lane * 8u);
             uint32_t e = kPairPending;
@@ -1678,7 +1763,9 @@
                 uint32_t idx[8];
 #pragma unroll
                 for (uint32_t q = 0; q < 4u; ++q) { idx[q] = (lv.x >> (8u * q)) & 0xFFu; idx[4u + q] = (lv.y >> (8u * q)) & 0xFFu; }
-                e = cell_pair_entry(idx, occ, lane);
+                uint32_t won;
+                e = cell_pair_entry(idx, occ, lane, remembered_direction(dirs, pcell), dirs.step, &won);
+                if (dirs.next && lane == 0u) dirs.next[pcell] = (uint8_t)won;
             }
             if (lane == 0u) pair_entries[pcell] = e;
             *reinterpret_cast<uint2 *>(colour_labels + (uint64_t)pcell * kCellColours + lane * 8u) = lv;
@@ -1889,9 +1976,17 @@
                        const uint32_t *work, const CellBounds *bounds, const CellBounds *sub_bounds, const Centroid *cent,
                        uint32_t k, const float4 *lab_table, uint64_t *masks, void *cell_work, void *colour_labels,
                        uint16_t *sub_table, int64_t *sums, uint32_t n_rows, uint32_t flags, unsigned long long *stats,
-                       hipStream_t st, const CubeTail *tail, const float *sub_affine, const CubeBalance *balance)
+                       hipStream_t st, const CubeTail *tail, const float *sub_affine, const CubeBalance *balance,
+                       const CubeDirections *directions)
 {
     const CubeTail tl = (tail && hist && n_rows <= 1u) ? *tail : CubeTail();
+    DirMemory dm;
+    static const bool directions_on = tools_env_int(KMG_TOOLS_ENV("KMG_DIRECTIONS"), 1) != 0;
+    if (directions && directions->state && hist && k <= 256u && !(flags & kCubeNoEntries) && directions_on) {
+        dm.next = directions->state + (directions->pass & 1u) * kCells;
+        dm.prev = directions->pass ? directions->state + ((directions->pass & 1u) ^ 1u) * kCells : nullptr;
+        dm.step = (kPairNeighbours * directions->pass) % 6u;
+    }
     const uint32_t kpad = (k + 63u) & ~63u;
     const bool with_sums = hist != nullptr;
     const uint32_t repl = with_sums ? cube_replicas(k) : 1u;
@@ -1918,7 +2013,7 @@
 #define KMG_SMALL(KP, S)                                                                                                    \
         hipLaunchKernelGGL((k_cube_small<KP, S>), dim3(g_small), dim3(kSmallBlock), lds, st, hist, agg, sub_agg, occ_bits,   \
                            work, bounds, sub_bounds, sub_affine, cent, k, lab_table, masks, (CellWork *)cell_work,            \
-                           (uint8_t *)colour_labels, sub_table, sums, n_rows, sflags, stats)
+                           (uint8_t *)colour_labels, sub_table, sums, n_rows, sflags, stats, dm)
         if (with_sums) { if (kp == 8u) KMG_SMALL(8, true); else if (kp == 16u) KMG_SMALL(16, true); else KMG_SMALL(32, true); }
         else           { if (kp == 8u) KMG_SMALL(8, false); else if (kp == 16u) KMG_SMALL(16, false); else KMG_SMALL(32, false); }
 #undef KMG_SMALL
@@ -1934,12 +2029,12 @@
                 hipLaunchKernelGGL((k_cube_scan<uint8_t, false>), dim3(g_scan2), dim3(kScanBlock), lds_scan2, st, hist, sub_agg, work, cent, k,
                                    lab_table, masks, (const CellWork *)cell_work, (uint8_t *)colour_labels, sub_table, sums, n_rows, repl2, flags);
             hipLaunchKernelGGL((k_cube_pairs<uint8_t>), dim3((flags & kCubeNoEntries) ? 1u : g_pairs2), dim3(kBlock), 0, st, work,
-                               with_sums ? 1 : 0, occ_bits, (const uint8_t *)colour_labels, sub_table, flags, sums, k, tl);
+                               with_sums ? 1 : 0, occ_bits, (const uint8_t *)colour_labels, sub_table, flags, sums, k, tl, dm);
             return hipGetLastError();
         }
         if (tl.acc_out)
             hipLaunchKernelGGL((k_cube_pairs<uint8_t>), dim3(1), dim3(kBlock), 0, st, work, 1, occ_bits,
-                               (const uint8_t *)colour_labels, sub_table, flags | kCubeNoEntries, sums, k, tl);
+                               (const uint8_t *)colour_labels, sub_table, flags | kCubeNoEntries, sums, k, tl, DirMemory());
         return hipGetLastError();
     }
     if (cube_single_launch(k, flags)) {
@@ -1951,14 +2046,14 @@
         if (with_sums)
             hipLaunchKernelGGL((k_cube_one<true>), dim3(kCells / kOneCells), dim3(kOneBlock), lds, st, hist, agg, sub_agg, occ_bits, work, bounds,
                                sub_bounds, sub_affine, cent, k, lab_table, masks, (uint8_t *)colour_labels, sub_table, sums, n_rows, flags, stats,
-                               balance ? balance->state : nullptr, balance ? balance->pass : 0u);
+                               balance ? balance->state : nullptr, balance ? balance->pass : 0u, dm);
         else
             hipLaunchKernelGGL((k_cube_one<false>), dim3(kCells / kOneCells), dim3(kOneBlock), lds, st, hist, agg, sub_agg, occ_bits, work, bounds,
                                sub_bounds, sub_affine, cent, k, lab_table, masks, (uint8_t *)colour_labels, sub_table, sums, n_rows, flags, stats,
-                               (uint16_t *)nullptr, 0u);
+                               (uint16_t *)nullptr, 0u, dm);
         if (tl.acc_out)
             hipLaunchKernelGGL((k_cube_pairs<uint8_t>), dim3(1), dim3(kBlock), 0, st, work, 1, occ_bits,
-                               (const uint8_t *)colour_labels, sub_table, flags | kCubeNoEntries, sums, k, tl);
+                               (const uint8_t *)colour_labels, sub_table, flags | kCubeNoEntries, sums, k, tl, DirMemory());
         return hipGetLastError();
     }
     static const uint32_t g_stage = env_grid("KMG_CUBE_GRID", 1536u), g_scan = env_grid("KMG_SCAN_GRID", kCubeGrid),
@@ -1977,7 +2072,7 @@
         hipLaunchKernelGGL((k_cube_scan<T, S>), dim3(g_scan), dim3(kScanBlock), lds_scan, st, hist, sub_agg, work, cent, k,   \
                            lab_table, masks, cw, (T *)colour_labels, sub_table, sums, n_rows, repl, flags);                 \
         hipLaunchKernelGGL((k_cube_pairs<T>), dim3((flags & kCubeNoEntries) ? 1u : g_pairs), dim3(kBlock), 0, st, work,   \
-                           S ? 1 : 0, occ_bits, (const T *)colour_labels, sub_table, flags, sums, k, tl);                   \
+                           S ? 1 : 0, occ_bits, (const T *)colour_labels, sub_table, flags, sums, k, tl, dm);               \
     } while (0)
     if (k <= 256) { if (with_sums) KMG_CUBE(uint8_t, true); else KMG_CUBE(uint8_t, false); }
     else          { if (with_sums) KMG_CUBE(uint16_t, true); else KMG_CUBE(uint16_t, false); }
@@ -1991,10 +2086,10 @@
     static const uint32_t g_pairs = env_grid("KMG_PAIRS_GRID", kCubeGrid);
     if (k <= 256)
         hipLaunchKernelGGL((k_cube_pairs<uint8_t>), dim3(g_pairs), dim3(kBlock), 0, st, work, work ? 1 : 0, occ_bits,
-                           (const uint8_t *)colour_labels, sub_table, 0u, (int64_t *)nullptr, k, CubeTail());
+                           (const uint8_t *)colour_labels, sub_table, 0u, (int64_t *)nullptr, k, CubeTail(), DirMemory());
     else
         hipLaunchKernelGGL((k_cube_pairs<uint16_t>), dim3(g_pairs), dim3(kBlock), 0, st, work, work ? 1 : 0, occ_bits,
-                           (const uint16_t *)colour_labels, sub_table, 0u, (int64_t *)nullptr, k, CubeTail());
+                           (const uint16_t *)colour_labels, sub_table, 0u, (int64_t *)nullptr, k, CubeTail(), DirMemory());
     return hipGetLastError();
 }
 
diff --git a/kmeans-gpu_amd/csrc/kmg_lloyd.hip b/kmeans-gpu_amd/csrc/kmg_lloyd.hip
--- a/kmeans-gpu_amd/csrc/kmg_lloyd.hip
+++ b/kmeans-gpu_amd/csrc/kmg_lloyd.hip
@@ -130,10 +130,10 @@
     if ((rc = ensure_bounds(s->p, S(stream))) != KMG_OK) return rc;
     ColourTable &t = s->tab;
     if (!t.d_hist) {
-        const size_t sizes[11] = {sizeof(uint32_t) << 24, sizeof(int64_t) * 4ull * kCells, sizeof(int64_t) * 4ull * kSubCells,
+        const size_t sizes[12] = {sizeof(uint32_t) << 24, sizeof(int64_t) * 4ull * kCells, sizeof(int64_t) * 4ull * kSubCells,
                                   (size_t)1 << 21, cube_work_bytes(), cube_masks_bytes(s->k),
                                   sizeof(uint32_t) * kWorkWords, (size_t)(s->k <= 256 ? 1 : 2) << 24, sub_table_bytes(),
-                                  sizeof(uint32_t) * (kCells + 1), cube_balance_bytes()};
+                                  sizeof(uint32_t) * (kCells + 1), cube_balance_bytes(), cube_directions_bytes()};
         size_t need = 0;
         for (size_t b : sizes) need += pad256(b);
         const hipError_t e = block_take(s->p, need, &t.blk, &t.blk_cap);
@@ -154,9 +154,12 @@
         t.d_sub = (uint16_t *)carve(t.blk, off, sizes[8]);
         t.share_buf = (uint32_t *)carve(t.blk, off, sizes[9]);
         t.d_balance = (uint16_t *)carve(t.blk, off, sizes[10]);
+        t.d_directions = (uint8_t *)carve(t.blk, off, sizes[11]);
     }
     t.d_work_share = nullptr;
     t.balance_work = nullptr;
+    HIP_TRY(hipMemsetAsync(t.d_balance, 0, cube_balance_bytes(), S(stream)));
+    HIP_TRY(hipMemsetAsync(t.d_directions, (int)kPairNoMemory, cube_directions_bytes(), S(stream)));
     t.rgba = nullptr;
     t.tables_valid = false;
     t.tie_valid = false;
@@ -398,13 +401,29 @@
 }
 KMG_ABI_CATCH
 
-static CubeBalance next_balance(ColourTable &t, const uint32_t *work)
-{
-    if (t.balance_work != work) { t.balance_work = work; t.balance_pass = 0; }
-    CubeBalance b;
-    b.state = t.d_balance;
-    b.pass = t.balance_pass++;
-    return b;
+struct CubeLoop {
+    CubeBalance balance;
+    CubeDirections directions;
+};
+
+static CubeLoop next_cube_pass(ColourTable &t, const uint32_t *work)
+{
+    if (t.balance_work != work) { t.balance_work = work; t.balance_pass = 0; t.directions_pass = 0; }
+    CubeLoop l;
+    l.balance.state = t.d_balance;
+    l.balance.pass = t.balance_pass;
+    l.directions.state = t.d_directions;
+    l.directions.pass = t.directions_pass;
+    return l;
+}
+
+static hipError_t cube_pass_done(ColourTable &t, hipError_t e, bool with_entries)
+{
+    if (e != hipSuccess) { t.balance_work = nullptr; return e; }
+    ++t.balance_pass;
+    t.entries_pass = -1;
+    if (with_entries) t.entries_pass = (int64_t)t.directions_pass++;
+    return e;
 }
 
 static int debug_refresh(kmg_lloyd *s, hipStream_t st, unsigned long long stage[8] = nullptr)
@@ -415,9 +434,12 @@
     if ((rc_ = side_flush(s, st)) != KMG_OK) return rc_;
     unsigned long long *d_stage = reinterpret_cast<unsigned long long *>(s->d_partials) + 4ull * s->k;
     HIP_TRY(hipMemsetAsync(s->d_partials, 0, sizeof(int64_t) * (4ull * s->k + 8ull), st));
+    CubeDirections dirs;
+    if (t.entries_valid && t.entries_pass >= 0) { dirs.state = t.d_directions; dirs.pass = (uint32_t)t.entries_pass; }
+    else t.entries_pass = -1;
     HIP_TRY(launch_cube(t.d_hist, t.d_agg, t.d_sub_agg, t.d_occ, t.d_work, s->p->d_bounds, s->p->d_sub_bounds, s->d_cent, s->k,
                         s->p->d_lab_table, t.d_masks, t.d_cell_work, t.d_colour_labels, t.d_sub, s->d_partials, 1u, 1u | (t.n_hot ? kCubeHot : 0u), d_stage, st,
-                        nullptr, affine_for(s->p, s->k, st)));
+                        nullptr, affine_for(s->p, s->k, st), nullptr, &dirs));
     t.entries_valid = true;
     if (stage) HIP_TRY(hipMemcpyAsync(stage, d_stage, 8 * sizeof(unsigned long long), hipMemcpyDeviceToHost, st));
     HIP_TRY(hipStreamSynchronize(st));
@@ -445,6 +467,7 @@
     if (t.entries_valid) return KMG_OK;
     HIP_TRY(launch_cube_entries(t.d_work_share ? t.d_work_share : t.d_work, t.d_occ, t.d_colour_labels, t.d_sub, s->k, st));
     t.entries_valid = true;
+    t.entries_pass = -1;
     return KMG_OK;
 }
 
@@ -458,11 +481,11 @@
         t.bound_by_init = false;
         int rc2;
         if ((rc2 = side_flush(s, st)) != KMG_OK) return rc2;
-        const CubeBalance bal = next_balance(t, t.d_work_share ? t.d_work_share : t.d_work);
-        PROF_LAUNCH(s, KMG_K_CUBE, st, launch_cube(t.d_hist, t.d_agg, t.d_sub_agg, t.d_occ, t.d_work_share ? t.d_work_share : t.d_work,
+        const CubeLoop loop = next_cube_pass(t, t.d_work_share ? t.d_work_share : t.d_work);
+        PROF_LAUNCH(s, KMG_K_CUBE, st, cube_pass_done(t, launch_cube(t.d_hist, t.d_agg, t.d_sub_agg, t.d_occ, t.d_work_share ? t.d_work_share : t.d_work,
                                                    s->p->d_bounds, s->p->d_sub_bounds, s->d_cent, s->k, s->p->d_lab_table, t.d_masks, t.d_cell_work,
                                                    t.d_colour_labels, t.d_sub, d_sums, 1u, t.n_hot ? kCubeHot : 0u, nullptr, st, nullptr,
-                                                   affine_for(s->p, s->k, st), &bal));
+                                                   affine_for(s->p, s->k, st), &loop.balance, &loop.directions), true));
         t.entries_valid = true;
         t.tables_valid = t.d_work_share == nullptr;
         return KMG_OK;
@@ -484,12 +507,13 @@
         tail.n_converged = s->d_nconv;
         static const bool tail_rides = tools_env_int(KMG_TOOLS_ENV("KMG_TAIL_ON_LABELS"), 1) != 0;
         const bool tail_on_labels = tail_rides && d_labels != nullptr && s->k <= 256u && cube_single_launch(s->k, t.n_hot ? kCubeHot : 0u);
-        const CubeBalance bal = next_balance(t, t.d_work_share ? t.d_work_share : t.d_work);
-        PROF_LAUNCH(s, KMG_K_CUBE, st, launch_cube(t.d_hist, t.d_agg, t.d_sub_agg, t.d_occ, t.d_work_share ? t.d_work_share : t.d_work,
+        const CubeLoop loop = next_cube_pass(t, t.d_work_share ? t.d_work_share : t.d_work);
+        PROF_LAUNCH(s, KMG_K_CUBE, st, cube_pass_done(t, launch_cube(t.d_hist, t.d_agg, t.d_sub_agg, t.d_occ, t.d_work_share ? t.d_work_share : t.d_work,
                                                    s->p->d_bounds, s->p->d_sub_bounds,
                                                    s->d_cent, s->k, s->p->d_lab_table, t.d_masks, t.d_cell_work, t.d_colour_labels, t.d_sub,
                                                    s->d_acc_int, 1u, (defer_entries ? kCubeNoEntries : 0u) | (t.n_hot ? kCubeHot : 0u), nullptr, st,
-                                                   tail_on_labels ? nullptr : &tail, affine_for(s->p, s->k, st), &bal));
+                                                   tail_on_labels ? nullptr : &tail, affine_for(s->p, s->k, st), &loop.balance, &loop.directions),
+                                                   !defer_entries));
         t.entries_valid = !defer_entries;
         if (tail_on_labels) {
             t.tables_valid = true;
@@ -507,6 +531,7 @@
                                                    s->d_cent, s->k, s->p->d_lab_table, t.d_masks, t.d_cell_work, t.d_colour_labels, t.d_sub,
                                                    d_sums, rows, t.n_hot ? kCubeHot : 0u, nullptr, st, nullptr, affine_for(s->p, s->k, st)));
         t.entries_valid = true;
+        t.entries_pass = -1;
     }
     t.tables_valid = t.d_work_share == nullptr;
     if (d_labels)
@@ -600,6 +625,7 @@
         h[i].C = chroma(h[i].a, h[i].b);
     }
     s->tab.tables_valid = false;
+    s->tab.directions_pass = 0;
     s->tab.bound_by_init = false;
     HIP_TRY(hipMemcpyAsync(s->d_cent, h.data(), sizeof(Centroid) * s->k, hipMemcpyHostToDevice, S(stream)));
     HIP_TRY(hipStreamSynchronize(S(stream)));
@@ -1104,10 +1130,11 @@
         if (update_first)
             PROF_LAUNCH(s, KMG_K_UPDATE, st, launch_update(d_acc4, s->k, s->p->opt.convergence, s->d_cent, s->d_nconv, st));
         HIP_TRY(hipMemsetAsync(d_acc4, 0, sizeof(int64_t) * 4ull * s->k, st));
-        const CubeBalance bal = next_balance(t, t.d_work);
-        PROF_LAUNCH(s, KMG_K_CUBE, st, launch_cube(t.d_hist, t.d_agg, t.d_sub_agg, t.d_occ, t.d_work, s->p->d_bounds, s->p->d_sub_bounds,
+        const CubeLoop loop = next_cube_pass(t, t.d_work);
+        PROF_LAUNCH(s, KMG_K_CUBE, st, cube_pass_done(t, launch_cube(t.d_hist, t.d_agg, t.d_sub_agg, t.d_occ, t.d_work, s->p->d_bounds, s->p->d_sub_bounds,
                                                    s->d_cent, s->k, s->p->d_lab_table, t.d_masks, t.d_cell_work, t.d_colour_labels, t.d_sub,
-                                                   d_acc4, 1u, t.n_hot ? kCubeHot : 0u, nullptr, st, nullptr, affine_for(s->p, s->k, st), &bal));
+                                                   d_acc4, 1u, t.n_hot ? kCubeHot : 0u, nullptr, st, nullptr, affine_for(s->p, s->k, st),
+                                                   &loop.balance, &loop.directions), true));
         return KMG_OK;
     };
     if ((rc = issue()) != KMG_OK) {
diff --git a/kmeans-gpu_amd/csrc/kmg_state.h b/kmeans-gpu_amd/csrc/kmg_state.h
--- a/kmeans-gpu_amd/csrc/kmg_state.h
+++ b/kmeans-gpu_amd/csrc/kmg_state.h
@@ -98,6 +98,9 @@
     uint16_t *d_balance = nullptr;
     const uint32_t *balance_work = nullptr;
     uint32_t balance_pass = 0;
+    uint8_t *d_directions = nullptr;
+    uint32_t directions_pass = 0;
+    int64_t entries_pass = -1;
     uint32_t *share_buf = nullptr;
     uint32_t *d_work_share = nullptr;
     bool tables_valid = false;
diff --git a/kmeans-gpu_amd/csrc/kmg_table.h b/kmeans-gpu_amd/csrc/kmg_table.h
--- a/kmeans-gpu_amd/csrc/kmg_table.h
+++ b/kmeans-gpu_amd/csrc/kmg_table.h
@@ -127,12 +127,20 @@
     uint32_t pass = 0;
 };
 size_t cube_balance_bytes();
+constexpr uint32_t kPairNoMemory = 255;
+constexpr uint32_t kPairNeighbours = 2;
+constexpr uint32_t kPairHeuristicOnly = 0xFFFFFFFFu;
+struct CubeDirections {
+    uint8_t *state = nullptr;
+    uint32_t pass = 0;
+};
+inline size_t cube_directions_bytes() { return 2u * (size_t)kCells; }
 hipError_t launch_cube(const uint32_t *hist, const int64_t *agg, const int64_t *sub_agg, const uint8_t *occ_bits,
                        const uint32_t *work, const CellBounds *bounds, const CellBounds *sub_bounds, const Centroid *cent,
                        uint32_t k, const float4 *lab_table, uint64_t *masks, void *cell_work, void *colour_labels,
                        uint16_t *sub_table, int64_t *sums, uint32_t n_rows, uint32_t flags, unsigned long long *stats,
                        hipStream_t st, const CubeTail *tail = nullptr, const float *sub_affine = nullptr,
-                       const CubeBalance *balance = nullptr);
+                       const CubeBalance *balance = nullptr, const CubeDirections *directions = nullptr);
 size_t sub_affine_bytes();
 hipError_t launch_sub_affine(const float4 *lab_table, const CellBounds *sub_bounds, float *affine, hipStream_t st);
 hipError_t launch_labels(const uint32_t *rgba, uint64_t n, const void *colour_labels,
```

Result: slower. 300.0 billion pixels/s (-2.8%).
